# Alibaba-Gemini-Lab/Gemini-SEAL

Measured on AMD Instinct MI355X. Metric: ciphertext multiply+relinearize/s (BFV N=2^15, 8 primes, bit-exact PARITY mode), higher is better.
Workload: dtype u64

## Files before the change

### gemini-seal_amd/csrc/api.cpp

```cpp
#include "../../include/sealhip.h"

#include <algorithm>
#include <cmath>
#include <cstdio>
#include <cstdlib>
#include <functional>
#include <vector>
#include <cstring>
#include <new>

#include "blake2xb.hpp"
#include "engine.hpp"
#include "evalmod_plan.hpp"
#include "homdft_plan.hpp"
#include "poly_plan.hpp"

using namespace sealhip;

namespace sealhip
{
    void wire_set_parms_id(Engine &e, int k, const std::uint64_t *id);
    void wire_peek(const void *bytes, std::size_t len, sealhip_ciphertext_info *info);
    void wire_load(Engine &e, const void *bytes, std::size_t len, sealhip_ciphertext_info *info, u64 *dst,
                   std::size_t capacity_words);
// ... 623 lines not shown
                          first ? "" : ", ", kv.first.c_str(), kv.second.launches, kv.second.ms, kv.second.units);
            out += buf;
            first = false;
        }
        out += "}";
        if (out.size() + 1 > capacity)
            throw std::invalid_argument("capacity too small");
        std::memcpy(json, out.c_str(), out.size() + 1);
    });
}

long sealhip_debug_ntt_table(sealhip_context *ctx, uint32_t prime_index, uint32_t kind, uint64_t *out_host,
                             size_t capacity)
{
    REQUIRE_PTR(ctx);
    REQUIRE_PTR(out_host);
    return guarded([&] {
        Engine &e = *ctx->engine;
        if (static_cast<int>(prime_index) >= e.n_primes() || kind > 3)
            throw std::invalid_argument("table index out of range");
        if (capacity < e.n)
            throw std::invalid_argument("capacity too small");
        const HostNttTables &tb = e.tables[prime_index];
        if (tb.fwd.empty())
            throw std::invalid_argument("this prime has no NTT tables");
        const std::vector<u64> v = tb.reference_table(static_cast<int>(kind));
        std::memcpy(out_host, v.data(), v.size() * sizeof(u64));
    });
}

long sealhip_debug_rns_constants(sealhip_context *ctx, uint32_t k, uint32_t which, uint64_t *out_host,
                                 size_t capacity, size_t *written)
{
    REQUIRE_PTR(ctx);
    REQUIRE_PTR(out_host);
    REQUIRE_PTR(written);
    return guarded([&] {
        Engine &e = *ctx->engine;
        check_level(e, k);
        const HostRnsTool &r = *e.level_host(static_cast<int>(k)).host_rns;
        std::vector<u64> v;
        switch (which)
        {
        case 0: v = r.Bsk; break;
        case 1: v = r.inv_prod_q_mod_Bsk; break;
        case 2: v = r.prod_q_mod_Bsk; break;
        case 3: v = r.inv_m_tilde_mod_Bsk; break;
        case 4: v = r.prod_B_mod_q; break;
        case 5: v = r.inv_q_last_mod_q; break;
        case 6: v = { r.inv_prod_q_mod_m_tilde, r.inv_prod_B_mod_m_sk, r.m_sk, r.gamma }; break;
        case 7: v = r.q_to_Bsk.matrix; break;
        case 8: v = r.B_to_q.matrix; break;
        case 9: v = r.q_to_Bsk.inv_punct; break;
        case 10: v = r.B_to_q.inv_punct; break;
        case 11: v = r.q_to_m_tilde.matrix; break;
        case 12: v = r.B_to_m_sk.matrix; break;
        default: throw std::invalid_argument("unknown constant selector");
        }
        if (capacity < v.size())
            throw std::invalid_argument("capacity too small");
        std::memcpy(out_host, v.data(), v.size() * sizeof(u64));
        *written = v.size();
    });
}

long sealhip_debug_bfv_multiply_plan(sealhip_context *ctx, uint32_t k, uint32_t size_a, uint32_t size_b, int32_t square,
                                     int32_t *out)
{
    REQUIRE_PTR(ctx);
    REQUIRE_PTR(out);
    return guarded([&] {
        Engine &e = *ctx->engine;
        check_level(e, k);
        if (size_a < 2 || size_b < 2 || size_a + size_b - 1 > 16)
            throw std::invalid_argument("encrypted1 or encrypted2 is not valid for encryption parameters");
        const BfvMulPlan p = plan_bfv_multiply(e, static_cast<int>(k), static_cast<int>(size_a), static_cast<int>(size_b),
                                               square != 0);
        const int32_t v[13] = { p.k, p.B, p.nB, p.square, p.redc_small, p.gather, p.defer, p.fused_tensor, p.tensor_apx,
                                p.lift_top, p.lift_kernel, p.floor_kernel, p.deferred_top };
        std::memcpy(out, v, sizeof v);
    });
}

long sealhip_debug_behz_dot_split(sealhip_context *ctx, uint32_t k, int32_t *out)
{
    REQUIRE_PTR(ctx);
    REQUIRE_PTR(out);
    return guarded([&] {
        Engine &e = *ctx->engine;
        check_level(e, k);
        if (e.scheme != 1)
            throw std::invalid_argument("BFV contexts only");
        if (e.device >= 0)
        {
            *out = e.level(static_cast<int>(k)).h_rns.dot_split;
            return;
        }
        const HostRnsTool &r = *e.level_host(static_cast<int>(k)).host_rns;
        const u64 max_q = *std::max_element(r.q.begin(), r.q.end()), max_b = *std::max_element(r.Bsk.begin(), r.Bsk.end());
        *out = bounds::behz_select_split(static_cast<int>(k), max_q, max_b);
    });
}

long sealhip_ntt_negacyclic_harvey_lazy(sealhip_context *ctx, uint64_t *data, size_t count, uint32_t k, uint32_t base)
{
    REQUIRE_PTR(ctx);
    REQUIRE_PTR(data);
    return guarded([&] { ntt_entry(ctx, data, count, k, base, false, 0); });
}
long sealhip_ntt_negacyclic_harvey(sealhip_context *ctx, uint64_t *data, size_t count, uint32_t k, uint32_t base)
{
    REQUIRE_PTR(ctx);
    REQUIRE_PTR(data);
    return guarded([&] { ntt_entry(ctx, data, count, k, base, false, kNttCanonical); });
}
long sealhip_inverse_ntt_negacyclic_harvey_lazy(sealhip_context *ctx, uint64_t *data, size_t count, uint32_t k,
                                                uint32_t base)
{
    REQUIRE_PTR(ctx);
    REQUIRE_PTR(data);
    return guarded([&] { ntt_entry(ctx, data, count, k, base, true, 0); });
}
long sealhip_inverse_ntt_negacyclic_harvey(sealhip_context *ctx, uint64_t *data, size_t count, uint32_t k,
                                           uint32_t base)
{
    REQUIRE_PTR(ctx);
    REQUIRE_PTR(data);
    return guarded([&] { ntt_entry(ctx, data, count, k, base, true, kNttCanonical); });
}

long sealhip_dyadic_product_coeffmod(sealhip_context *ctx, const uint64_t *a, const uint64_t *b, size_t count,
                                     uint32_t k, uint32_t base, uint64_t *result)
{
    REQUIRE_PTR(ctx);
    REQUIRE_PTR(a);
    REQUIRE_PTR(b);
    REQUIRE_PTR(result);
    return guarded([&] { poly_entry(ctx, PolyOp::Dyadic, a, b, 0, result, count, k, base); });
}
long sealhip_multiply_poly_scalar_coeffmod(sealhip_context *ctx, const uint64_t *a, size_t count, uint32_t k,
                                           uint32_t base, uint64_t scalar, uint64_t *result)
{
    REQUIRE_PTR(ctx);
    REQUIRE_PTR(a);
    REQUIRE_PTR(result);
    return guarded([&] { poly_entry(ctx, PolyOp::Scalar, a, a, scalar, result, count, k, base); });
}
long sealhip_add_poly_coeffmod(sealhip_context *ctx, const uint64_t *a, const uint64_t *b, size_t count, uint32_t k,
                               uint32_t base, uint64_t *result)
{
    REQUIRE_PTR(ctx);
    REQUIRE_PTR(a);
    REQUIRE_PTR(b);
    REQUIRE_PTR(result);
    return guarded([&] { poly_entry(ctx, PolyOp::Add, a, b, 0, result, count, k, base); });
}
long sealhip_sub_poly_coeffmod(sealhip_context *ctx, const uint64_t *a, const uint64_t *b, size_t count, uint32_t k,
                               uint32_t base, uint64_t *result)
{
    REQUIRE_PTR(ctx);
    REQUIRE_PTR(a);
    REQUIRE_PTR(b);
    REQUIRE_PTR(result);
    return guarded([&] { poly_entry(ctx, PolyOp::Sub, a, b, 0, result, count, k, base); });
}
long sealhip_negate_poly_coeffmod(sealhip_context *ctx, const uint64_t *a, size_t count, uint32_t k, uint32_t base,
// ... 3225 lines not shown
```

### gemini-seal_amd/csrc/engine.hpp

```cpp
#pragma once

#include <hip/hip_runtime.h>

#include <cstddef>
#include <array>
#include <atomic>
#include <cstdint>
#include <functional>
#include <map>
#include <memory>
#include <mutex>
#include <stdexcept>
#include <string>
#include <cstdlib>
#include <vector>

#include "devmath.hpp"
#include "ntt_bounds.hpp"
#include "ntt_select.hpp"
#include "hostmath.hpp"
#include "pool_scratch.hpp"
#include "held_workspace.hpp"
struct sealhip_kswitch_key;

// ... 280 lines not shown
        int n_primes() const
        {
            return static_cast<int>(tables.size());
        }
        LevelTools &level(int k);
        LevelTools &level_host(int k);
        LevelTools &level_rescale(int k);
        const std::uint32_t *galois_table(std::uint32_t elt);
        void ws_reset() const
        {
            Lane &l = lane();
            l.ws_used = l.ws_floor;
        }
        u64 *ws_alloc(std::size_t words) const;
        void ws_reserve(std::size_t bytes) const;
        RowMap map_for(int k, unsigned base);
        int rows_for(int k, unsigned base);
    };

    struct HipError : std::runtime_error
    {
        hipError_t code;
        HipError(hipError_t c, const char *what) : std::runtime_error(what), code(c)
        {}
    };
#define SEALHIP_CHECK(expr)                                                                          \
    do                                                                                               \
    {                                                                                                \
        hipError_t _e = (expr);                                                                      \
        if (_e != hipSuccess)                                                                        \
            throw ::sealhip::HipError(_e, (std::string(#expr) + ": " + hipGetErrorString(_e)).c_str()); \
    } while (0)
    inline void check(hipError_t err, const char *what)
    {
        if (err != hipSuccess)
            throw HipError(err, (std::string(what) + ": " + hipGetErrorString(err)).c_str());
    }

    inline std::size_t pad256(std::size_t words)
    {
        return (words * sizeof(u64) + 255) & ~static_cast<std::size_t>(255);
    }
    struct Carver
    {
        char *base;
        std::size_t at = 0;
        u64 *take(std::size_t words)
        {
            u64 *p = reinterpret_cast<u64 *>(base + at);
            at += pad256(words);
            return p;
        }
    };

    constexpr int kThreads = 256;
    inline unsigned grid_for(std::size_t work_items, std::size_t max_blocks = 256u * 16u)
    {
        const std::size_t blocks = (work_items + kThreads - 1) / kThreads;
        return static_cast<unsigned>(blocks < max_blocks ? (blocks ? blocks : 1) : max_blocks);
    }

    struct ProfScope
    {
        const Engine &e;
        ProfScope(const Engine &eng, const char *tag, double units) : e(eng)
        {
            if (e.lane().prof_on)
                e.prof_begin(tag, units);
        }
        ~ProfScope()
        {
            if (e.lane().prof_on)
                e.prof_end();
        }
    };

    hipError_t ntt_init_kernels();
    hipError_t ntt_butterfly_rate(const Engine &e, int kind, int prime_id, double *butterflies_per_s);
    hipError_t launch_ntt(const Engine &e, u64 *data, std::size_t nrows, const RowMap &map, bool inverse, int flags);
    bool ntt_can_gather(const Engine &e);
    bool ntt_strict_top_done_ok(const Engine &e, const RowMap &map);
    hipError_t launch_ntt_gather(const Engine &e, u64 *data, std::size_t nrows, const RowMap &map, const NttSource &src,
                                 int flags);

    enum class PolyOp
    {
        Dyadic,
        Add,
        Sub,
        Negate,
        Scalar,
        Mod63
    };
    hipError_t launch_poly_op(const Engine &e, PolyOp op, const u64 *a, const u64 *b, u64 scalar, u64 *r,
                              std::size_t nrows, const RowMap &map);
    hipError_t launch_tensor_product(const Engine &e, const u64 *a, int sa, std::size_t a_stride, const u64 *b, int sb,
                                     std::size_t b_stride, u64 *out, std::size_t out_stride, std::size_t count,
                                     const RowMap &map, bool square = false);
    hipError_t launch_fill_rows(const Engine &e, u64 *dst, const u64 *row_values, int rows, std::size_t count);
    constexpr int kDotGroup = bounds::kDotGroupTerms;
    struct DotTerms
    {
        const u64 *a[kDotGroup];
        const u64 *b[kDotGroup];
        int n;
    };
    hipError_t launch_tensor_dot(const Engine &e, const DotTerms &terms, std::size_t a_stride, std::size_t b_stride, u64 *out01,
                                 std::size_t out01_stride, u64 *out2, std::size_t out2_stride, std::size_t count,
                                 const RowMap &map, bool reduce_on_load, bool add_partial);
    constexpr int kLinGroup = bounds::kLinGroupTerms, kLinTile = bounds::kLinTileSums;
    struct LinTerms
    {
        const u64 *x[kLinGroup];
        int n;
    };
    hipError_t launch_lincomb(const Engine &e, const LinTerms &terms, int size, std::size_t x_stride, const u64 *w,
                              std::size_t w_sum_stride, const u64 *constant, int const_mode, u64 *out, std::size_t out_sum_stride,
                              int n_sums, std::size_t count, const RowMap &map, bool add_partial, std::size_t flag_sum_stride);
    constexpr int kLinLevelsTile = bounds::kLinLevelsTileSums;
    struct LinLevelTerms
    {
        const u64 *x[kLinGroup];
        unsigned char rows[kLinGroup];
        unsigned char size[kLinGroup];
        int n;
    };
    hipError_t launch_lincomb_levels(const Engine &e, const LinLevelTerms &terms, int size, std::size_t out_stride, const u64 *w,
                                     std::size_t w_sum_stride, const u64 *constant, int const_mode, u64 *out,
                                     std::size_t out_sum_stride, int n_sums, std::size_t count, const RowMap &map,
                                     bool add_partial, std::size_t flag_sum_stride);
    hipError_t launch_poly_tables(const Engine &e, int k, const u64 *coeffs, std::size_t n_coeffs, std::size_t ms, u64 *w,
                                  u64 *constant);
    constexpr int kPutWords = 256;
    hipError_t launch_put_words(const Engine &e, u64 *dst, const u64 *words, std::size_t n);
    hipError_t launch_copy_rows(const Engine &e, const u64 *src, std::size_t src_poly_stride, u64 *dst,
                                std::size_t dst_poly_stride, std::size_t npolys, int rows);

    hipError_t launch_fastbconv_m_tilde(const Engine &e, const RnsDev *d, const RnsDev &h, const u64 *in,
                                        std::size_t in_stride, u64 *out, std::size_t out_stride, std::size_t count);
    hipError_t launch_sm_mrq(const Engine &e, const RnsDev *d, const RnsDev &h, const u64 *in, std::size_t in_stride,
                             u64 *out, std::size_t out_stride, std::size_t count);
    constexpr int kBehzGeneric = 32;
    constexpr int kBehzStepwise = 64;
    struct BfvMulPlan
    {
        int k, B, nB;
        bool square;
        bool redc_small;
        bool gather;
        bool defer;
        bool fused_tensor;
        bool tensor_apx;
        bool lift_top;
        int lift_kernel;
        int floor_kernel;
        int deferred_top;
    };
    BfvMulPlan plan_bfv_multiply(Engine &e, int k, int sa, int sb, bool square);

    bool bfv_lift_can_apply_top(const Engine &e, int k, bool redc_small);
    hipError_t launch_bfv_lift(const Engine &e, const RnsDev *d, const RnsDev &h, const u64 *in, std::size_t in_stride,
                               u64 *out, std::size_t out_stride, std::size_t count, const BfvMulPlan &plan);
    hipError_t launch_fast_floor(const Engine &e, const RnsDev *d, const RnsDev &h, const u64 *in,
                                 std::size_t in_stride, u64 *out, std::size_t out_stride, std::size_t count,
                                 int mul_t);
    hipError_t launch_fastbconv_sk(const Engine &e, const RnsDev *d, const RnsDev &h, const u64 *in,
                                   std::size_t in_stride, u64 *out, std::size_t out_stride, std::size_t count);
    hipError_t launch_bfv_floor_sk(const Engine &e, const RnsDev *d, const RnsDev &h, const u64 *in,
                                   std::size_t in_stride, u64 *out, std::size_t out_stride, std::size_t count,
                                   const BfvMulPlan &plan);
    bool ntt_can_defer_top(const Engine &e, int k);
    bool ntt_can_fuse_moddown(const Engine &e, int k, u64 p_special);
    hipError_t launch_intt_from(const Engine &e, u64 *data, const u64 *src, std::size_t src_poly_stride, std::size_t nrows,
                                const RowMap &map, int flags);
    hipError_t launch_intt_tensor(const Engine &e, u64 *data, const u64 *x, std::size_t item_stride, std::size_t poly_stride,
                                  int kb, std::size_t nrows, const RowMap &map, int flags, bool square = false);
    hipError_t launch_divround_bfv(const Engine &e, const RnsDev *d, const RnsDev &h, const u64 *in,
                                   std::size_t in_stride, u64 *out, std::size_t out_stride, std::size_t count,
                                   int out_rows);
    hipError_t launch_rescale_pre(const Engine &e, const RnsDev *d, const RnsDev &h, u64 *last,
                                  std::size_t last_stride, u64 *temp, std::size_t temp_stride, std::size_t count);
    hipError_t launch_rescale_post(const Engine &e, const RnsDev *d, const RnsDev &h, const u64 *in,
                                   std::size_t in_stride, const u64 *temp, std::size_t temp_stride, u64 *out,
                                   std::size_t out_stride, std::size_t count);

    enum class CtLinearOp
    {
        Add,
        Sub,
        Negate,
        MulPlain
    };
    hipError_t launch_ct_linear(const Engine &e, CtLinearOp op, const u64 *a, int sa, const u64 *b, int sb,
                                std::size_t b_item_stride, u64 *out, std::size_t count, const RowMap &map);
    hipError_t launch_nonzero_words(const Engine &e, const u64 *data, std::size_t item_stride, std::size_t words,
                                    std::size_t count, unsigned *flags);
    hipError_t launch_nonzero_tail(const Engine &e, const u64 *ct, std::size_t item_words, std::size_t skip_words,
                                   std::size_t count, unsigned *flags);
    struct SinkScope
    {
        Engine &e;
        Lane &l;
        bool on;
        size_t count;
        bool cleared = false;
        SinkScope(Engine &eng, size_t n) : e(eng), l(eng.lane()), on(l.tsink != nullptr), count(n)
        {
            if (on && count > l.tsink_cap)
                throw std::invalid_argument("the transparency sink is smaller than this batch");
        }
        void clear()
        {
            if (on && !cleared && count)
                SEALHIP_CHECK(hipMemsetAsync(l.tsink, 0, count * sizeof(unsigned), l.stream));
            cleared = true;
            l.tsink_base = 0;
        }
        void begin()
        {
            clear();
            if (on)
                l.tsink_cur = l.tsink;
        }
        void arm()
        {
            begin();
        }
        void read_pass(const u64 *result, uint32_t size, size_t poly_words, size_t n)
        {
            clear();
            if (on && size >= 2 && n)
                check(launch_nonzero_tail(e, result, poly_words * size, poly_words, n, l.tsink), "transparency");
        }
        ~SinkScope()
        {
            l.tsink_cur = l.tsink_arm = nullptr;
            l.tsink_base = 0;
        }
    };
    hipError_t launch_out_of_range(const Engine &e, const u64 *ct, std::size_t item_words, std::size_t count,
                                   const RowMap &map, unsigned *flags);
    hipError_t launch_plain_lift(const Engine &e, const u64 *plain, std::size_t plain_stride, u64 *out, std::size_t nplains,
                                 const RowMap &map, u64 t);
    hipError_t launch_plain_lift_centered(const Engine &e, const u64 *plain, std::size_t coeff_count, std::size_t plain_stride,
                                          u64 *out, std::size_t nplains, const RowMap &map, u64 t);
    hipError_t launch_galois(const Engine &e, const u64 *in, u64 *out, std::size_t nrows, const RowMap &map,
                             std::uint32_t elt, const std::uint32_t *table );

    hipError_t launch_ks_modup(const Engine &e, const KsDev *d, const KsDev &h, const u64 *coeff,
                               std::size_t coeff_stride, u64 *ext, std::size_t ext_stride,
                               std::size_t ext_digit_stride, std::size_t count, int only_digit);
    hipError_t launch_ks_mac(const Engine &e, const KsDev *d, const KsDev &h, const u64 *target,
                             std::size_t target_stride, const u64 *ext, std::size_t ext_stride,
                             std::size_t ext_digit_stride, const u64 *key, u64 *prod, std::size_t prod_stride,
                             std::size_t count, int j0 = 0, int j1 = -1);
    hipError_t launch_ks_moddown_pre(const Engine &e, const KsDev *d, const KsDev &h, const u64 *prod,
                                     std::size_t prod_stride, u64 *temp, std::size_t temp_stride, std::size_t npolys);
    hipError_t launch_ks_moddown_bfv(const Engine &e, const KsDev *d, const KsDev &h, const u64 *prod,
                                     std::size_t prod_stride, u64 *ct, std::size_t ct_item_stride, std::size_t npolys,
                                     bool top_deferred, const u64 *c0_src = nullptr, std::size_t c0_stride = 0);
    hipError_t launch_ks_moddown_post(const Engine &e, const KsDev *d, const KsDev &h, u64 *prod,
                                      std::size_t prod_stride, const u64 *temp, std::size_t temp_stride, u64 *ct,
                                      std::size_t ct_item_stride, std::size_t npolys, int add_into_ct,
                                      const u64 *c0_src = nullptr, std::size_t c0_stride = 0);
    hipError_t launch_ks_rescale_fold(const Engine &e, const KsRescaleDev *d, const KsRescaleDev &h, const u64 *base,
                                      std::size_t base_stride, u64 *acc, std::size_t acc_stride, std::size_t npolys);
    hipError_t launch_ks_moddown_rescale_pre(const Engine &e, const KsRescaleDev *d, const KsRescaleDev &h, const u64 *acc,
                                             std::size_t acc_stride, u64 *temp, std::size_t npolys);
    hipError_t launch_ks_moddown_rescale_post(const Engine &e, const KsRescaleDev *d, const KsRescaleDev &h, const u64 *base,
                                              std::size_t base_stride, const u64 *acc, std::size_t acc_stride, const u64 *temp,
                                              u64 *out, std::size_t npolys);

    constexpr int kHoistMaxElts = 16;
    struct HoistElts
    {
        int n;
        std::uint32_t elt[kHoistMaxElts];
        const std::uint32_t *table[kHoistMaxElts];
        const u64 *key[kHoistMaxElts];
    };
    hipError_t launch_hoist_mac(const Engine &e, const KsDev *d, const KsDev &h, const u64 *target,
                                std::size_t target_stride, const u64 *ext, std::size_t ext_stride,
                                std::size_t ext_digit_stride, const HoistElts &elts, u64 *prod, std::size_t prod_stride,
                                std::size_t count);
    hipError_t launch_hoist_galois_c0(const Engine &e, const u64 *ct, std::size_t ct_stride, u64 *out, std::size_t count,
                                      const RowMap &map_q, const HoistElts &elts, bool ntt_form);
    struct HoistDotElts
    {
        int n;
        const std::uint32_t *table[kHoistMaxElts];
        const u64 *key[kHoistMaxElts];
        const u64 *w[kHoistMaxElts];
    };
    hipError_t launch_hoist_dot_mac(const Engine &e, const KsDev *d, const KsDev &h, const u64 *target,
                                    std::size_t target_stride, const u64 *ext, std::size_t ext_stride,
                                    std::size_t ext_digit_stride, const HoistDotElts &elts, std::size_t w_sum_stride, u64 *acc,
                                    std::size_t acc_stride, std::size_t count, std::size_t n_sums, bool add);
    hipError_t launch_hoist_dot_base(const Engine &e, const u64 *cn, const HoistDotElts &elts, std::size_t w_sum_stride,
                                     u64 *out, std::size_t out_sum_stride, int k, std::size_t count, std::size_t n_sums,
                                     bool add);

    struct HoistGiantElts
    {
        int n;
        const std::uint32_t *table[kHoistMaxElts];
        const u64 *key[kHoistMaxElts];
        const u64 *inb[kHoistMaxElts];
        const u64 *ext[kHoistMaxElts];
        const u64 *accj[kHoistMaxElts];
    };
    hipError_t launch_hoist_giant_mac(const Engine &e, const KsDev *d, const KsDev &h, const HoistGiantElts &elts,
                                      std::size_t inb_stride, std::size_t ext_stride, std::size_t ext_digit_stride,
                                      std::size_t accj_stride, u64 *acc, std::size_t acc_stride, std::size_t count, bool add);
    struct HoistGiantBases
    {
        int n;
        const std::uint32_t *table[kHoistMaxElts];
        const u64 *base[kHoistMaxElts];
    };
    hipError_t launch_hoist_giant_base(const Engine &e, const HoistGiantBases &elts, u64 *out, int k, std::size_t count,
                                       bool add);

    struct HostBatchIO
    {
        struct In
        {
            const u64 *const *ptrs;
            std::size_t words;
        };
        struct Out
        {
            u64 *const *ptrs;
            std::size_t words;
        };
        std::vector<In> in;
        std::vector<Out> out;
        std::size_t tmp_words = 0;
    };
// ... 276 lines not shown
```

### gemini-seal_amd/csrc/keyswitch.hip

```cpp
#include <cstdlib>
#include "engine.hpp"

namespace sealhip
{
    namespace
    {
        __device__ __forceinline__ const u64 *modup_block(const KsDev *d, int j)
        {
            const int rows = d->k + d->nsp;
            return d->modup + static_cast<std::size_t>(j) * (2 * d->nsp + rows * d->nsp);
        }

        __global__ __launch_bounds__(kThreads) void ks_modup_kernel(const KsDev *__restrict__ d,
                                                                    const PrimeDev *__restrict__ primes,
                                                                    const u64 *__restrict__ coeff,
                                                                    std::size_t coeff_stride, u64 *__restrict__ ext,
                                                                    std::size_t ext_stride,
                                                                    std::size_t ext_digit_stride, std::size_t count,
                                                                    int logn, int only_digit)
        {
            const std::size_t i = blockIdx.x * static_cast<std::size_t>(blockDim.x) + threadIdx.x;
            const std::size_t item = i >> logn;
            if (item >= count)
                return;
// ... 85 lines not shown
            const int my_digit = r < k ? r / nsp : -1;
            const u64 *pext = ext + item * ext_stride + static_cast<std::size_t>(r) * N + c;
            const u64 *pkey = key + static_cast<std::size_t>(rns_idx) * N + c;
            const std::size_t key_comp = static_cast<std::size_t>(n_total) * N;
            u64 lo0 = 0, hi0 = 0, lo1 = 0, hi1 = 0;
            for (int j = j0; j < j1; j++)
            {
                const u64 x = j == my_digit ? target[item * target_stride + static_cast<std::size_t>(r) * N + c]
                                            : pext[static_cast<std::size_t>(j) * ext_digit_stride];
                const u64 k0 = pkey[(2 * static_cast<std::size_t>(j)) * key_comp];
                const u64 k1 = pkey[(2 * static_cast<std::size_t>(j) + 1) * key_comp];
                mac128(lo0, hi0, x, k0);
                mac128(lo1, hi1, x, k1);
            }
            const PrimeDev &P = primes[rns_idx];
            u64 *pp = prod + item * prod_stride + static_cast<std::size_t>(r) * N + c;
            pp[0] = barrett_reduce_128(lo0, hi0, P.p, P.cr0, P.cr1);
            pp[static_cast<std::size_t>(rows) * N] = barrett_reduce_128(lo1, hi1, P.p, P.cr0, P.cr1);
        }

        template <int ND>
        __global__ __launch_bounds__(kThreads) void ks_mac_items_kernel(const KsDev *__restrict__ d,
                                                                        const PrimeDev *__restrict__ primes,
                                                                        const u64 *__restrict__ target,
                                                                        std::size_t target_stride,
                                                                        const u64 *__restrict__ ext,
                                                                        std::size_t ext_stride,
                                                                        std::size_t ext_digit_stride,
                                                                        const u64 *__restrict__ key,
                                                                        u64 *__restrict__ prod, std::size_t prod_stride,
                                                                        std::size_t count, int logn, std::size_t group)
        {
            const std::size_t N = static_cast<std::size_t>(1) << logn;
            const int k = d->k, nsp = d->nsp, rows = k + nsp, n_total = d->n_total;
            const std::size_t i = blockIdx.x * static_cast<std::size_t>(blockDim.x) + threadIdx.x;
            const std::size_t c = i & (N - 1);
            const std::size_t rr = i >> logn;
            const int r = static_cast<int>(rr % rows);
            const std::size_t item0 = (rr / rows) * group;
            if (item0 >= count)
                return;
            const std::size_t item1 = item0 + group < count ? item0 + group : count;
            const int rns_idx = d->row_prime[r];
            const int my_digit = r < k ? r / nsp : -1;
            const std::size_t row_off = static_cast<std::size_t>(r) * N + c;
            const u64 *pkey = key + static_cast<std::size_t>(rns_idx) * N + c;
            const std::size_t key_comp = static_cast<std::size_t>(n_total) * N;
            u64 k0[ND], k1[ND], x[ND], xn[ND];
#pragma unroll
            for (int j = 0; j < ND; j++)
            {
                k0[j] = pkey[(2 * static_cast<std::size_t>(j)) * key_comp];
                k1[j] = pkey[(2 * static_cast<std::size_t>(j) + 1) * key_comp];
            }
            auto load_x = [&](u64(&dst)[ND], std::size_t item) {
#pragma unroll
                for (int j = 0; j < ND; j++)
                    dst[j] = j == my_digit ? target[item * target_stride + row_off]
                                           : ext[item * ext_stride + static_cast<std::size_t>(j) * ext_digit_stride + row_off];
            };
            load_x(x, item0);
            const PrimeDev &P = primes[rns_idx];
            const u64 p = P.p, cr0 = P.cr0, cr1 = P.cr1;
            for (std::size_t item = item0; item < item1; item++)
            {
                if (item + 1 < item1)
                    load_x(xn, item + 1);
                u64 lo0 = 0, hi0 = 0, lo1 = 0, hi1 = 0;
#pragma unroll
                for (int j = 0; j < ND; j++)
                {
                    mac128(lo0, hi0, x[j], k0[j]);
                    mac128(lo1, hi1, x[j], k1[j]);
                }
                u64 *pp = prod + item * prod_stride + row_off;
                store_stream(pp, barrett_reduce_128(lo0, hi0, p, cr0, cr1));
                store_stream(pp + static_cast<std::size_t>(rows) * N, barrett_reduce_128(lo1, hi1, p, cr0, cr1));
#pragma unroll
                for (int j = 0; j < ND; j++)
                    x[j] = xn[j];
            }
        }

        __global__ __launch_bounds__(kThreads) void ks_moddown_pre_kernel(const KsDev *__restrict__ d,
                                                                          const PrimeDev *__restrict__ primes,
                                                                          const u64 *__restrict__ prod,
                                                                          std::size_t prod_stride,
                                                                          u64 *__restrict__ temp,
                                                                          std::size_t temp_stride, std::size_t npolys,
                                                                          int logn)
        {
            const std::size_t i = blockIdx.x * static_cast<std::size_t>(blockDim.x) + threadIdx.x;
            const std::size_t poly = i >> logn;
            if (poly >= npolys)
                return;
            const std::size_t N = static_cast<std::size_t>(1) << logn;
            const std::size_t c = i & (N - 1);
            const int k = d->k, nsp = d->nsp;
            const u64 *sp = prod + poly * prod_stride + static_cast<std::size_t>(k) * N + c;
            u64 *pt = temp + poly * temp_stride + c;
            if (nsp == 1)
            {
                const PrimeDev &S = primes[d->row_prime[k]];
                const u64 v = neg_mod(barrett_reduce_63(sp[0], S.p, S.cr1), S.p);
                for (int q = 0; q < k; q++)
                {
                    const PrimeDev &Q = primes[d->row_prime[q]];
                    pt[q * N] = barrett_reduce_63(v, Q.p, Q.cr1);
                }
                return;
            }
            for (int q = 0; q < k; q++)
            {
                const PrimeDev &Q = primes[d->row_prime[q]];
                u64 lo = 0, hi = 0;
                for (int j = 0; j < nsp; j++)
                {
                    const u64 pj = primes[d->row_prime[k + j]].p;
                    const u64 y = mulmod_shoup(sp[j * N], d->inv_hat[j], d->inv_hat_shoup[j], pj);
                    mac128(lo, hi, y, d->neg_hat[q * nsp + j]);
                }
                pt[q * N] = barrett_reduce_128(lo, hi, Q.p, Q.cr0, Q.cr1);
            }
        }

        __global__ __launch_bounds__(kThreads) void ks_moddown_post_kernel(const KsDev *__restrict__ d,
                                                                           const PrimeDev *__restrict__ primes,
                                                                           u64 *__restrict__ prod,
                                                                           std::size_t prod_stride,
                                                                           const u64 *__restrict__ temp,
                                                                           std::size_t temp_stride,
                                                                           u64 *__restrict__ ct,
                                                                           std::size_t ct_item_stride,
                                                                           std::size_t npolys, int logn,
                                                                           int add_into_ct, const u64 *__restrict__ c0_src,
                                                                           std::size_t c0_stride, unsigned *__restrict__ tflags)
        {
            const std::size_t N = static_cast<std::size_t>(1) << logn;
            const int k = d->k;
            const std::size_t i = blockIdx.x * static_cast<std::size_t>(blockDim.x) + threadIdx.x;
            const std::size_t c = i & (N - 1);
            const std::size_t rr = i >> logn;
            const int q = static_cast<int>(rr % k);
            const std::size_t poly = rr / k;
            if (poly >= npolys)
                return;
            const PrimeDev &Q = primes[d->row_prime[q]];
            u64 *pp = prod + poly * prod_stride + static_cast<std::size_t>(q) * N + c;
            const u64 v = mulmod_shoup(*pp + temp[poly * temp_stride + static_cast<std::size_t>(q) * N + c], d->invP[q],
                                       d->invP_shoup[q], Q.p);
            if (add_into_ct)
            {
                u64 *pc = ct + (poly >> 1) * ct_item_stride + ((poly & 1) * static_cast<std::size_t>(k) + q) * N + c;
                u64 w;
                if (!c0_src)
                    w = add_mod(v, *pc, Q.p);
                else
                    w = (poly & 1) ? v : add_mod(v, c0_src[(poly >> 1) * c0_stride + static_cast<std::size_t>(q) * N + c], Q.p);
                *pc = w;
                if (poly & 1)
                    note_nonzero(tflags, poly >> 1, w);
            }
            else
                *pp = v;
        }

// ... 144 lines not shown
                u64 z[ND1];
#pragma unroll
                for (int a = 0; a < ND1; a++)
                    z[a] = rescale_z(d, primes, a, dp[a * N], slo, shi);
                const u64 v = shi;
                for (int r = 0; r < k - 1; r++)
                {
                    const PrimeDev &Q = primes[r];
                    const u64 *hat = d->hat + static_cast<std::size_t>(r) * ND1;
                    u64 lo = d->neg_half[r], hi = 0;
#pragma unroll
                    for (int a = 0; a < ND1; a++)
                        mac128(lo, hi, z[a], hat[a]);
                    mac128(lo, hi, v, d->neg_D[r]);
                    pt[r * N] = barrett_reduce_128(lo, hi, Q.p, Q.cr0, Q.cr1);
                }
            }
            else
            {
                for (int a = 0; a < nd1; a++)
                    rescale_z(d, primes, a, dp[a * N], slo, shi);
                const u64 v = shi;
                for (int r = 0; r < k - 1; r++)
                {
                    const PrimeDev &Q = primes[r];
                    const u64 *hat = d->hat + static_cast<std::size_t>(r) * nd1;
                    u64 lo = d->neg_half[r], hi = 0, s0 = 0, s1 = 0;
                    for (int a = 0; a < nd1; a++)
                        mac128(lo, hi, rescale_z(d, primes, a, dp[a * N], s0, s1), hat[a]);
                    mac128(lo, hi, v, d->neg_D[r]);
                    pt[r * N] = barrett_reduce_128(lo, hi, Q.p, Q.cr0, Q.cr1);
                }
            }
        }

        __global__ __launch_bounds__(kThreads) void ks_moddown_rescale_post_kernel(const KsRescaleDev *__restrict__ d,
                                                                                   const PrimeDev *__restrict__ primes,
                                                                                   const u64 *__restrict__ base,
                                                                                   std::size_t base_stride,
                                                                                   const u64 *__restrict__ acc,
                                                                                   std::size_t acc_stride,
                                                                                   const u64 *__restrict__ temp, u64 *__restrict__ out,
                                                                                   std::size_t npolys, int logn,
                                                                                   unsigned *__restrict__ tflags)
        {
            const std::size_t N = static_cast<std::size_t>(1) << logn;
            const int k = d->k, kk = k - 1;
            const std::size_t i = blockIdx.x * static_cast<std::size_t>(blockDim.x) + threadIdx.x;
            const std::size_t c = i & (N - 1);
            const std::size_t rr = i >> logn;
            const int r = static_cast<int>(rr % kk);
            const std::size_t poly = rr / kk;
            if (poly >= npolys)
                return;
            const PrimeDev &Q = primes[r];
            const std::size_t row = static_cast<std::size_t>(r) * N + c;
            const u64 b = base[(poly >> 1) * base_stride + (poly & 1) * static_cast<std::size_t>(k) * N + row];
            const u64 s = mul_add_mod(b, d->P_mod_q[r], acc[poly * acc_stride + row], Q.p, Q.cr0, Q.cr1);
            const std::size_t o = poly * static_cast<std::size_t>(kk) * N + row;
            const u64 w = mulmod_shoup(sub_mod(s, temp[o], Q.p), d->invD[r], d->invD_shoup[r], Q.p);
            store_stream(out + o, w);
            if (poly & 1)
                note_nonzero(tflags, poly >> 1, w);
        }

        inline unsigned blocks_for(std::size_t lanes)
        {
            return static_cast<unsigned>((lanes + kThreads - 1) / kThreads);
        }
    }

    hipError_t launch_ks_modup(const Engine &e, const KsDev *d, const KsDev &, const u64 *coeff,
                               std::size_t coeff_stride, u64 *ext, std::size_t ext_stride,
                               std::size_t ext_digit_stride, std::size_t count, int only_digit)
    {
        if (!count)
            return hipSuccess;
        ProfScope prof(e, "ks_modup", 0);
        ks_modup_kernel<<<blocks_for(count << e.logn), kThreads, 0, e.lane().stream>>>(
            d, e.d_primes, coeff, coeff_stride, ext, ext_stride, ext_digit_stride, count, e.logn, only_digit);
        return hipGetLastError();
    }

    hipError_t launch_ks_mac(const Engine &e, const KsDev *d, const KsDev &h, const u64 *target,
                             std::size_t target_stride, const u64 *ext, std::size_t ext_stride,
                             std::size_t ext_digit_stride, const u64 *key, u64 *prod, std::size_t prod_stride,
                             std::size_t count, int j0, int j1)
    {
        if (!count)
            return hipSuccess;
        if (j1 < 0)
            j1 = h.nd;
        if (j0 < 0 || j0 > j1 || j1 > h.nd)
            return hipErrorInvalidValue;
        const bool all_digits = j0 == 0 && j1 == h.nd;
        const u64 *tg = target;
        const std::size_t lanes = (count * static_cast<std::size_t>(h.k + h.nsp)) << e.logn;
        ProfScope prof(e, "ks_mac", 0);
        const std::size_t key_bytes = (2ull * h.nd * (h.k + h.nsp)) << (e.logn + 3);
        const std::size_t cap = key_bytes > (std::size_t(48) << 20) ? 64 : 16;
        std::size_t mac_group = 8;
        for (std::size_t g = cap; g > 8; g >>= 1)
            if ((((count + g - 1) / g * static_cast<std::size_t>(h.k + h.nsp)) << e.logn) / kThreads >= 4096)
            {
                mac_group = g;
                break;
            }
        const std::size_t groups = (count + mac_group - 1) / mac_group;
        const std::size_t glanes = (groups * static_cast<std::size_t>(h.k + h.nsp)) << e.logn;
#define SEALHIP_KS_MAC(ND)                                                                                          \
    case ND:                                                                                                        \
        ks_mac_items_kernel<ND><<<blocks_for(glanes), kThreads, 0, e.lane().stream>>>(                                     \
            d, e.d_primes, tg, target_stride, ext, ext_stride, ext_digit_stride, key, prod, prod_stride, count,    \
            e.logn, mac_group);                                                                                     \
        break;
        switch (count >= 16 && all_digits ? h.nd : 0)
        {
            SEALHIP_KS_MAC(1)
            SEALHIP_KS_MAC(2)
            SEALHIP_KS_MAC(3)
            SEALHIP_KS_MAC(4)
            SEALHIP_KS_MAC(5)
            SEALHIP_KS_MAC(6)
            SEALHIP_KS_MAC(7)
            SEALHIP_KS_MAC(8)
            SEALHIP_KS_MAC(9)
            SEALHIP_KS_MAC(10)
            SEALHIP_KS_MAC(11)
            SEALHIP_KS_MAC(12)
            SEALHIP_KS_MAC(13)
            SEALHIP_KS_MAC(14)
            SEALHIP_KS_MAC(15)
            SEALHIP_KS_MAC(16)
        default:
            ks_mac_kernel<<<blocks_for(lanes), kThreads, 0, e.lane().stream>>>(d, e.d_primes, tg, target_stride, ext, ext_stride,
                                                                        ext_digit_stride, key, prod, prod_stride, count,
                                                                        e.logn, j0, j1);
        }
#undef SEALHIP_KS_MAC
        return hipGetLastError();
    }

    hipError_t launch_ks_moddown_pre(const Engine &e, const KsDev *d, const KsDev &, const u64 *prod,
                                     std::size_t prod_stride, u64 *temp, std::size_t temp_stride, std::size_t npolys)
    {
        if (!npolys)
            return hipSuccess;
        ProfScope prof(e, "ks_moddown_pre", 0);
        ks_moddown_pre_kernel<<<blocks_for(npolys << e.logn), kThreads, 0, e.lane().stream>>>(
            d, e.d_primes, prod, prod_stride, temp, temp_stride, npolys, e.logn);
        return hipGetLastError();
    }

    hipError_t launch_ks_moddown_bfv(const Engine &e, const KsDev *d, const KsDev &h, const u64 *prod,
                                     std::size_t prod_stride, u64 *ct, std::size_t ct_item_stride, std::size_t npolys,
                                     bool top_deferred, const u64 *c0_src, std::size_t c0_stride)
    {
        if (!npolys)
            return hipSuccess;
        const std::size_t lanes = npolys << (e.logn - 1);
        ProfScope prof(e, "ks_moddown_bfv", 0);
#define SEALHIP_MODDOWN_BFV(DEFER_, ONE_)                                                                            \
    ks_moddown_bfv_kernel<DEFER_, ONE_><<<blocks_for(lanes), kThreads, 0, e.lane().stream>>>(                              \
        d, e.d_primes, prod, prod_stride, ct, ct_item_stride, npolys, e.logn, c0_src, c0_stride, e.lane().tsink_arm)
        if (top_deferred && h.nsp == 1)
            SEALHIP_MODDOWN_BFV(true, true);
        else if (top_deferred)
            SEALHIP_MODDOWN_BFV(true, false);
        else if (h.nsp == 1)
            SEALHIP_MODDOWN_BFV(false, true);
        else
            SEALHIP_MODDOWN_BFV(false, false);
#undef SEALHIP_MODDOWN_BFV
        return hipGetLastError();
    }

    hipError_t launch_ks_moddown_post(const Engine &e, const KsDev *d, const KsDev &h, u64 *prod,
                                      std::size_t prod_stride, const u64 *temp, std::size_t temp_stride, u64 *ct,
                                      std::size_t ct_item_stride, std::size_t npolys, int add_into_ct, const u64 *c0_src,
                                      std::size_t c0_stride)
    {
        if (!npolys)
            return hipSuccess;
        const std::size_t lanes = (npolys * static_cast<std::size_t>(h.k)) << e.logn;
        ProfScope prof(e, "ks_moddown_post", 0);
        ks_moddown_post_kernel<<<blocks_for(lanes), kThreads, 0, e.lane().stream>>>(
            d, e.d_primes, prod, prod_stride, temp, temp_stride, ct, ct_item_stride, npolys, e.logn, add_into_ct, c0_src, c0_stride,
            add_into_ct ? e.lane().tsink_arm : nullptr);
        return hipGetLastError();
    }

    hipError_t launch_ks_rescale_fold(const Engine &e, const KsRescaleDev *d, const KsRescaleDev &, const u64 *base,
// ... 51 lines not shown
```

### gemini-seal_amd/csrc/ntt.hip

```cpp
#include <cstdlib>
#include <stdexcept>

#include "ntt_half.hpp"

namespace sealhip
{
    namespace
    {
        constexpr int kTileBitsMax = 13;

        __device__ __forceinline__ int pad_index(int l)
        {
            return l + (l >> 4);
        }

        template <int DIR>
        __global__ __launch_bounds__(512, 4) void ntt_pass_kernel(u64 *__restrict__ data,
                                                               const PrimeDev *__restrict__ primes, RowMap map,
                                                               NttPass ps)
        {
            extern __shared__ u64 lds[];
            const int tid = threadIdx.x;
            const int nthreads = blockDim.x;
            const int t = ps.t, c = ps.c, b_lo = ps.b_lo, logn = ps.logn;
// ... 421 lines not shown
                               reinterpret_cast<const void *>(&butterfly_rate_kernel<4>), reinterpret_cast<const void *>(&butterfly_rate_kernel<5>) };
        if ((err = hipFuncSetAttribute(fns[kind], hipFuncAttributeMaxDynamicSharedMemorySize, static_cast<int>(lds))) != hipSuccess)
        {
            (void)hipEventDestroy(a);
            (void)hipEventDestroy(b);
            (void)hipFree(sink);
            return err;
        }
        const auto launch = [&](int n) {
            switch (kind)
            {
            case 0: butterfly_rate_kernel<0><<<blocks, 512, lds, st>>>(sink, P, n); break;
            case 1: butterfly_rate_kernel<1><<<blocks, 512, lds, st>>>(sink, P, n); break;
            case 2: butterfly_rate_kernel<2><<<blocks, 512, lds, st>>>(sink, P, n); break;
            case 3: butterfly_rate_kernel<3><<<blocks, 512, lds, st>>>(sink, P, n); break;
            case 4: butterfly_rate_kernel<4><<<blocks, 512, lds, st>>>(sink, P, n); break;
            default: butterfly_rate_kernel<5><<<blocks, 512, lds, st>>>(sink, P, n); break;
            }
        };
        launch(iters / 8);
        (void)hipEventRecord(a, st);
        launch(iters);
        launch(iters);
        (void)hipEventRecord(b, st);
        err = hipStreamSynchronize(st);
        float ms = 0;
        if (err == hipSuccess)
            err = hipEventElapsedTime(&ms, a, b);
        (void)hipEventDestroy(a);
        (void)hipEventDestroy(b);
        (void)hipFree(sink);
        if (err != hipSuccess)
            return err;
        *butterflies_per_s = 2.0 * blocks * 512.0 * iters * 32.0 / (ms / 1e3);
        return hipGetLastError();
    }

    hipError_t ntt_init_kernels()
    {
        const int max_lds = ((1 << kTileBitsMax) + (1 << (kTileBitsMax - 4))) * 8;
        hipError_t err = hipFuncSetAttribute(reinterpret_cast<const void *>(&ntt_pass_kernel<0>),
                                             hipFuncAttributeMaxDynamicSharedMemorySize, max_lds);
        if (err != hipSuccess)
            return err;
        err = hipFuncSetAttribute(reinterpret_cast<const void *>(&ntt_pass_kernel<1>),
                                  hipFuncAttributeMaxDynamicSharedMemorySize, max_lds);
        if (err == hipSuccess)
            err = ntt_fwd_half_init();
        if (err == hipSuccess)
            err = ntt_inv_half_init();
        return err;
    }

    bool ntt_can_defer_top(const Engine &e, int k)
    {
        return e.use_half_kernel && e.logn >= 14 && e.logn <= 16 && k <= 32;
    }

    bool ntt_can_fuse_moddown(const Engine &e, int k, u64 p_special)
    {
        if (!fp64_enabled() || !ntt_can_gather(e) || e.logn < 15 || p_special >= kFpPrimeBound)
            return false;
        for (int r = 0; r < k; r++)
            if (e.key_moduli[r] >= kFpPrimeBound)
                return false;
        return true;
    }

    bool ntt_strict_top_done_ok(const Engine &e, const RowMap &map)
    {
        if (!e.use_half_kernel || e.logn < 14 || e.logn > 16 || exact_fwd())
            return false;
        for (int r = 0; r < map.rows; r++)
            if (map.prime[r] != kSkipRow && !bounds::fwd_dense_admits(e.tables[map.prime[r]].p, e.logn))
                return false;
        return true;
    }

    bool ntt_can_gather(const Engine &e)
    {
        return e.use_half_kernel && e.logn >= 14 && e.logn <= 16;
    }

    hipError_t launch_ntt_gather(const Engine &e, u64 *data, size_t nrows, const RowMap &map, const NttSource &src,
                                 int flags)
    {
        if (!ntt_can_gather(e))
            return hipErrorInvalidValue;
        if (e.mode_strict)
            flags |= kNttStrict;
        if (nrows == 0)
            return hipSuccess;
        return ntt_fwd_half(e, data, nrows, map, flags, src);
    }

    hipError_t launch_intt_from(const Engine &e, u64 *data, const u64 *src, std::size_t src_poly_stride, size_t nrows,
                                const RowMap &map, int flags)
    {
        if (!(e.use_half_kernel && e.logn >= 14 && e.logn <= 16))
            return hipErrorInvalidValue;
        if (nrows == 0)
            return hipSuccess;
        return ntt_inv_half(e, data, nrows, map, flags, src, src_poly_stride);
    }

    hipError_t launch_intt_tensor(const Engine &e, u64 *data, const u64 *x, std::size_t item_stride, std::size_t poly_stride,
                                  int kb, size_t nrows, const RowMap &map, int flags, bool square)
    {
        if (!(e.use_half_kernel && e.logn >= 14 && e.logn <= 16) || map.rows != 3 * kb)
            return hipErrorInvalidValue;
        if (nrows == 0)
            return hipSuccess;
        return ntt_inv_tensor(e, data, nrows, map, flags, x, item_stride, poly_stride, kb, square);
    }

    hipError_t launch_ntt(const Engine &e, u64 *data, size_t nrows, const RowMap &map, bool inverse, int flags)
    {
        if (nrows == 0)
            return hipSuccess;
        if (e.mode_strict)
            flags |= kNttStrict;
        if (e.use_half_kernel && e.logn >= 14 && e.logn <= 16)
            return inverse ? ntt_inv_half(e, data, nrows, map, flags) : ntt_fwd_half(e, data, nrows, map, flags, NttSource{});
        if (e.logn > kTileBitsMax)
            return hipErrorInvalidValue;
        const NttPlan plan = plan_ntt(e.logn, inverse, flags);
        return inverse ? launch_dir<1>(e, data, nrows, map, plan) : launch_dir<0>(e, data, nrows, map, plan);
    }
}
```

### gemini-seal_amd/csrc/ntt_bounds.hpp

```cpp
#pragma once
#include <cstdint>

namespace sealhip
{
    namespace bounds
    {
        using u64 = unsigned long long;
        using u128 = unsigned __int128;

        constexpr int kMinHalfLogn = 14, kMaxHalfLogn = 16;
        constexpr int kMaxPrimeBits = 61;
        constexpr u128 kWord = static_cast<u128>(1) << 64;
        constexpr long double kFpLimit = 9007199254740992.0L;

        constexpr u64 max_prime_of_bits(int bits)
        {
            return (bits >= 64 ? ~u64(0) : (u64(1) << bits) - 1);
        }
        constexpr u64 max_ntt_prime_of_bits(int bits, int logn)
        {
            return bits > logn + 1 ? (u64(1) << bits) - (u64(1) << (logn + 1)) + 1 : 0;
        }

        constexpr int kInvLazyProductMult = 4;
// ... 61 lines not shown
                          inv_lazy_prime_bits(16, 1) == 60,
                      "dense lazy inverse: primes below 2^60 in every shape");
        static_assert(inv_lazy_max_shift(16, 1) == 3, "dense lazy inverse: values entering a layer are below 8p");

        constexpr int kFwdApxLevel = 2;
        static_assert(kFwdApxLevel == 1 || kFwdApxLevel == 2, "approximate-quotient form");
        constexpr int quotient_shortfall(int level)
        {
            return level == 0 ? 1 : (level == 1 ? 2 : 3);
        }
        constexpr int kFwdApxGrowth = quotient_shortfall(kFwdApxLevel) + 1;
        constexpr u128 fwd_int_peak(int logn, u64 p, int in_mult, bool apx, bool skip_last_barrett)
        {
            const u128 g = static_cast<u128>(apx ? kFwdApxGrowth : 2) * p;
            u128 bound = static_cast<u128>(in_mult) * p, peak = bound;
            for (int l = 0; l < logn; l++)
            {
                u128 u = bound;
                if (l == logn - 1 && !skip_last_barrett)
                    u = static_cast<u128>(2) * p;
                const u128 out = u + g;
                peak = out > peak ? out : peak;
                bound = out;
            }
            return peak;
        }
        constexpr int fwd_lazy_prime_bits(int logn)
        {
            int bits = 0;
            for (int b = 1; b <= kMaxPrimeBits; b++)
                if (fwd_int_peak(logn, max_prime_of_bits(b), 2, true, true) < kWord)
                    bits = b;
            return bits;
        }
        static_assert(kFwdApxLevel != 1 || (fwd_lazy_prime_bits(14) == 58 && fwd_lazy_prime_bits(16) == 58),
                      "level 1: kNttAnyRep / kNttApprox / unreduced mod-up: primes below 2^58 (50p at log n = 16)");
        static_assert(kFwdApxLevel != 2 || (fwd_lazy_prime_bits(14) == 58 && fwd_lazy_prime_bits(15) == 58 && fwd_lazy_prime_bits(16) == 57),
                      "level 2: 58p / 62p below 2^64 for primes below 2^58 at log n = 14 / 15; 66p at log n = 16: below 2^57");
        constexpr bool fwd_lazy_admits(u64 p, int logn)
        {
            return logn >= kMinHalfLogn && logn <= kMaxHalfLogn && p <= max_prime_of_bits(fwd_lazy_prime_bits(logn));
        }
        constexpr int kCanonInMult = 4;
        constexpr int fwd_canon_output_mult(int logn)
        {
            return kCanonInMult + kFwdApxGrowth * logn;
        }
        constexpr bool fwd_canon_admits(u64 p, int logn)
        {
            return logn >= kMinHalfLogn && logn <= kMaxHalfLogn && fwd_lazy_admits(p, logn) &&
                   fwd_int_peak(logn, p, kCanonInMult, true, true) < kWord;
        }
        constexpr int fwd_apx_output_mult(int logn, bool anyrep)
        {
            return anyrep ? 2 + kFwdApxGrowth * logn : 2 + kFwdApxGrowth;
        }

        constexpr int kFwdDenseInMult = 4;
        constexpr bool fwd_dense_reduce_before_round(int r)
        {
            return r == 2 || r == 3;
        }
        constexpr int fwd_dense_peak_mult(int logn)
        {
            int b = kFwdDenseInMult + 2, peak = b;
            for (int r = 1; r <= 4; r++)
            {
                if (fwd_dense_reduce_before_round(r))
                    b = 2;
                const int layers = r <= 3 ? 4 : logn - 13;
                for (int l = 0; l < layers; l++)
                    b += 2;
                peak = b > peak ? b : peak;
            }
            return peak;
        }
        constexpr bool fwd_dense_admits(u64 p, int logn)
        {
            return logn >= kMinHalfLogn && logn <= kMaxHalfLogn && p < (u64(1) << 60) &&
                   small_quot_admits(p, fwd_dense_peak_mult(logn)) && static_cast<u128>(fwd_dense_peak_mult(logn)) * p <= kWord;
        }
        static_assert(fwd_dense_peak_mult(14) == 14 && fwd_dense_peak_mult(15) == 14 && fwd_dense_peak_mult(16) == 16,
                      "dense forward schedule: 14p after round 1, at most 16p after the final round at N = 2^16");

        constexpr bool tensor_redc_ok(u64 p, int operand_mult, int np)
        {
            const u128 ob = static_cast<u128>(operand_mult) * p;
            if (ob > (static_cast<u128>(1) << 61) || np > 2)
                return false;
            return (ob - 1) * (ob - 1) * np <= static_cast<u128>(p) * kWord;
        }
        constexpr int tensor_prime_bits(int operand_mult)
        {
            int bits = 0;
            for (int b = 1; b <= kMaxPrimeBits; b++)
                if (tensor_redc_ok(max_prime_of_bits(b), operand_mult, 2))
                    bits = b;
            return bits;
        }
        constexpr int kTensorPrimeBits4p = tensor_prime_bits(4);
        constexpr int kTensorPrimeBits2p = tensor_prime_bits(2);
        static_assert(kTensorPrimeBits4p == 59, "fused tensor product on [0, 4p) operands: ciphertext primes below 2^59");
        static_assert(kTensorPrimeBits2p == 60, "... on [0, 2p) operands (kNttReduceOut rows): the 60-bit Bsk primes");
        constexpr bool tensor_admits_4p(u64 p)
        {
            return p <= max_prime_of_bits(kTensorPrimeBits4p);
        }
        constexpr bool tensor_admits_2p(u64 p)
        {
            return p <= max_prime_of_bits(kTensorPrimeBits2p);
        }
        constexpr int kTensorPrimeBitsApx = tensor_prime_bits(fwd_apx_output_mult(kMaxHalfLogn, false));
        static_assert(kTensorPrimeBitsApx == (kFwdApxLevel == 2 ? 57 : 58), "fused tensor product on approximate-quotient rows");
        constexpr bool tensor_admits_apx(u64 p)
        {
            return p <= max_prime_of_bits(kTensorPrimeBitsApx);
        }

        constexpr long double kFpSlack = 1.0L + 0x1p-40L;
        constexpr long double fp_mul_bound(long double y, long double p)
        {
            return 0.5L * p + 3.0L * 0x1p-53L * y * p * kFpSlack;
        }
        constexpr long double fp_reduce_bound(long double x, long double p)
        {
            return 0.5L * p + x * 0x1p-51L + 1.0L;
        }
        constexpr bool fp_fwd_reduce_before_layer(int i)
        {
            return i == 5 || i == 10;
        }
        constexpr long double fp_fwd_peak(int logn, long double p, long double in_bound)
        {
            long double b = in_bound, peak = in_bound;
            b = b + fp_mul_bound(b, p);
            peak = b > peak ? b : peak;
            b = fp_reduce_bound(b, p);
            for (int i = 0; i < logn - 1; i++)
            {
                if (fp_fwd_reduce_before_layer(i))
                    b = fp_reduce_bound(b, p);
                b = b + fp_mul_bound(b, p);
                peak = b > peak ? b : peak;
            }
            return peak;
        }
        constexpr bool fp_inv_reduce_after_layer(int T, int l)
        {
            return l % 4 == 1 && l != T - 1;
        }
        constexpr long double fp_inv_peak(int T, long double p)
        {
            long double b = 2.0L * p, peak = b;
            for (int l = 0; l < T; l++)
            {
                const long double s = 2.0L * b;
                peak = s > peak ? s : peak;
                const long double r = fp_mul_bound(s, p);
                b = s > r ? s : r;
                if (fp_inv_reduce_after_layer(T, l))
                    b = fp_reduce_bound(b, p);
            }
            return peak;
        }
        constexpr int fp_prime_bits()
        {
// ... 268 lines not shown
```

### gemini-seal_amd/csrc/ntt_fwd.hip

```cpp
#include <cstring>
#include <utility>

#include "ntt_half.hpp"

namespace sealhip
{
    namespace
    {
        template <int STRICT>
        constexpr int kApx = STRICT == kSchedApprox ? bounds::kFwdApxLevel : 0;
        constexpr int kFinalZeroPairs = 2;
        template <int T, int STRICT>
        constexpr int kFinalApx = (kApx<STRICT> == 2 && (T - 12) == 2) ? 1 : kApx<STRICT>;
        template <int STRICT>
        __device__ __forceinline__ u64 fwd_addend(u64 two_p, u64 neg_p)
        {
            if constexpr (STRICT != kSchedApprox)
                return two_p;
            u64 a = two_p << 1;
            asm("" : "+s"(a));
            return a;
        }


// ... 462 lines not shown
                        };
                        top(lo[i].x, hi[i].x);
                        top(lo[i].y, hi[i].y);
                    }
                }
                if constexpr (REDUCE == kTreatNegSpecial)
                {
#pragma unroll
                    for (int i = 0; i < kLoadBatch; i++)
                    {
                        const auto red = [&](u64 v) {
                            if constexpr (STRICT == kSchedFp64)
                            {
                                const double P = fp_of(aux_p), r = fp_canonical(fp_from_u64(v), P, fp_of(aux_cr1));
                                return fp_bits(r != 0.0 ? P - r : 0.0);
                            }
                            const u64 r = barrett_reduce_63(v, aux_p, aux_cr1);
                            return r ? aux_p - r : 0;
                        };
                        lo[i].x = red(lo[i].x);
                        lo[i].y = red(lo[i].y);
                        hi[i].x = red(hi[i].x);
                        hi[i].y = red(hi[i].y);
                    }
                }
                if constexpr (REDUCE == kTreatBarrett || REDUCE == kTreatCondSub)
                {
                    const u64 p = STRICT == kSchedFp64 ? static_cast<u64>(fp_of(two_p)) : 0 - neg_p;
                    const auto red = [&](u64 v) {
                        if constexpr (REDUCE == kTreatCondSub)
                            return v >= p ? v - p : v;
                        else
                            return barrett_reduce_63(v, p, cr1);
                    };
#pragma unroll
                    for (int i = 0; i < kLoadBatch; i++)
                    {
                        lo[i].x = red(lo[i].x);
                        lo[i].y = red(lo[i].y);
                        hi[i].x = red(hi[i].x);
                        hi[i].y = red(hi[i].y);
                    }
                }
#pragma unroll
                for (int i = 0; i < kLoadBatch; i += 2)
                {
                    const int s = (batch * kLoadBatch + i) * 2;
                    u64 u[4] = {lo[i].x, lo[i].y, lo[i + 1].x, lo[i + 1].y};
                    u64 y[4] = {hi[i].x, hi[i].y, hi[i + 1].x, hi[i + 1].y};
                    if constexpr (STRICT == kSchedFp64)
                    {
#pragma unroll
                        for (int j = 0; j < 4; j++)
                        {
                            if constexpr (REDUCE != kTreatNegSpecial && REDUCE != kTreatNegSpecialTop && REDUCE != kTreatModDownStore)
                            {
                                u[j] = fp_bits(fp_from_u64(u[j]));
                                y[j] = fp_bits(fp_from_u64(y[j]));
                            }
                            fp_butterfly_fwd(u[j], y[j], W1.x, fp_of(two_p), fp_of(neg_p));
                            x[s + j] = HALF ? y[j] : u[j];
                        }
                        continue;
                    }
                    const u64 w[4] = {W1.x, W1.x, W1.x, W1.x}, ws[4] = {W1.y, W1.y, W1.y, W1.y};
                    if (STRICT == kSchedHarvey)
                    {
#pragma unroll
                        for (int j = 0; j < 4; j++)
                            u[j] = u[j] >= two_p ? u[j] - two_p : u[j];
                    }
                    if constexpr (kApx<STRICT> == 2)
                        butterflies_fwd_apx2<true, 4>(u, y, w, ws, neg_p, fwd_addend<STRICT>(two_p, neg_p), zp.z);
                    else
                        butterflies_fwd_hs<true, 4, kApx<STRICT>>(u, y, w, ws, neg_p, fwd_addend<STRICT>(two_p, neg_p));
#pragma unroll
                    for (int j = 0; j < 4; j++)
                        x[s + j] = HALF ? y[j] : u[j];
                }
                __builtin_amdgcn_sched_barrier(0);
            }
        }

        template <int T>
        __device__ __forceinline__ void h_store_rows(const u64 (&x)[32], u64 *__restrict__ halfp, int tid)
        {
            const int jb = Arr<T, 1>::tid_index(tid);
#pragma unroll
            for (int s = 0; s < 32; s += 2)
                store_nt(halfp + jb + Arr<T, 1>::slot_index(s), x[s], x[s + 1]);
        }

        template <int T>
        __device__ __forceinline__ void h_store_moddown(const u64 (&x)[32], int tid, const u64 *__restrict__ prod_half,
                                                        u64 *__restrict__ ct_half, const u64 *__restrict__ c0_half, bool add_ct,
                                                        u64 inv_p, u64 inv_p_shoup, u64 p, unsigned *__restrict__ tflag)
        {
            const int jb = Arr<T, 1>::tid_index(tid);
            u64 nz = 0;
#pragma unroll
            for (int b = 0; b < 32; b += 8)
            {
                ulonglong2 pr[4], cc[4];
#pragma unroll
                for (int i = 0; i < 4; i++)
                {
                    const int off = jb + Arr<T, 1>::slot_index(b + 2 * i);
                    pr[i] = *reinterpret_cast<const ulonglong2 *>(prod_half + off);
                    if (c0_half)
                        cc[i] = *reinterpret_cast<const ulonglong2 *>(c0_half + off);
                    else if (add_ct)
                        cc[i] = *reinterpret_cast<const ulonglong2 *>(ct_half + off);
                }
#pragma unroll
                for (int i = 0; i < 4; i++)
                {
                    const int off = jb + Arr<T, 1>::slot_index(b + 2 * i);
                    u64 v0 = mulmod_shoup(pr[i].x + x[b + 2 * i], inv_p, inv_p_shoup, p);
                    u64 v1 = mulmod_shoup(pr[i].y + x[b + 2 * i + 1], inv_p, inv_p_shoup, p);
                    if (c0_half || add_ct)
                    {
                        v0 = add_mod(v0, cc[i].x, p);
                        v1 = add_mod(v1, cc[i].y, p);
                    }
                    store_nt(ct_half + off, v0, v1);
                    nz |= v0 | v1;
                }
            }
            note_nonzero(tflag, 0, nz);
        }

        template <int LOGN, int STRICT, int REDUCE>
        __global__ __launch_bounds__(1 << (LOGN - 6), 4) void ntt_fwd_half_kernel(
            u64 *__restrict__ data, const PrimeDev *__restrict__ primes, RowMap map, std::size_t nrows, int flags,
            unsigned *__restrict__ tickets, unsigned *__restrict__ timeout_flag, unsigned spin_limit, NttSource src,
            std::size_t chunk, LiveSlots live)
        {
            constexpr int T = LOGN - 1;
            constexpr int N = 1 << LOGN;
            extern __shared__ u64 lds[];
            const int wave_base = __builtin_amdgcn_readfirstlane(static_cast<int>(threadIdx.x) & ~63);
            int half, position;
            std::size_t poly;
            if (!half_block_map(blockIdx.x, nrows / map.rows, live.n, chunk, poly, position, half,
                                (flags & kNttPolyMajor) ? ((flags >> 16) & 0xFF) : 0))
                return;
            const std::size_t row = poly * map.rows + live.slot[position];
            const unsigned short pid = map.prime[row % map.rows];
            const PrimeDev P = primes[pid];
            constexpr bool FP = STRICT == kSchedFp64;
            const u64 p = P.p, two_p = FP ? fp_bits(P.p_d) : P.two_p, rdp = P.rdp;
            const u64 *tw = FP ? reinterpret_cast<const u64 *>(P.fwd_d) : P.fwd;
            u64 *rowp = data + (row << LOGN);
            u64 x[32];

            const u64 neg_p = FP ? fp_bits(P.pinv_d) : 0 - p;
            const u64 *srcp = rowp;
            if (src.base[0])
            {
                const unsigned short code = src.code[row % map.rows];
                if (code != kSkipRow)
                {
                    const int b = code >> 15;
                    srcp = src.base[b] + (row / map.rows) * src.poly_stride[b] +
                           (static_cast<std::size_t>(code & 0x3FFF) << LOGN);
                }
            }
            if constexpr (REDUCE == kTreatReduceOutTopDone)
            {
                const int jb1 = Arr<T, 1>::tid_index(fresh_tid(wave_base));
#pragma unroll
                for (int s = 0; s < 32; s += 2)
                {
                    const ulonglong2 v = *reinterpret_cast<const ulonglong2 *>(rowp + (half << T) + jb1 + Arr<T, 1>::slot_index(s));
                    x[s] = v.x;
                    x[s + 1] = v.y;
                }
            }
            else if (half)
                h_load_top<T, STRICT, 1, REDUCE>(x, srcp, tw, fresh_tid(wave_base), two_p, neg_p, P.cr1, src.aux_p, src.aux_cr1, src.aux_top);
            else
                h_load_top<T, STRICT, 0, REDUCE>(x, srcp, tw, fresh_tid(wave_base), two_p, neg_p, P.cr1, src.aux_p, src.aux_cr1, src.aux_top);
            const int gbase = half << T;
            u64 w0[kIL], ws0[kIL];
            RoundStage<T, 1, STRICT, true, 0>::load(w0, ws0, tw, gbase, N);
            if constexpr (FP)
                fp_reduce_all(x, two_p, neg_p);
            ZeroPairs zp;
            if constexpr (kApx<STRICT> == 2)
                zp.init();
            RoundPipe<T, 1, STRICT, true>::run(x, w0, ws0, tw, gbase, N, two_p, neg_p, zp);
            const int jb2 = gbase + Arr<T, 2>::tid_index(fresh_tid(wave_base));
            RoundStage<T, 2, STRICT, false, 0>::load(w0, ws0, tw, jb2, N);
            __builtin_amdgcn_sched_barrier(0);
            h_exchange<T, 1, 2>(x, lds, fresh_tid(wave_base));
            if (fresh_tid(wave_base) == 0 && tickets && !(flags & kNttDebugNoSignal))
                __hip_atomic_fetch_add(&tickets[row], 1u, __ATOMIC_RELAXED, __HIP_MEMORY_SCOPE_AGENT);
            if constexpr (kApx<STRICT> == 2)
                zp.init();
            RoundPipe<T, 2, STRICT, false>::run(x, w0, ws0, tw, jb2, N, two_p, neg_p, zp);
            const int jb3 = gbase + Arr<T, 3>::tid_index(fresh_tid(wave_base));
            RoundStage<T, 3, STRICT, false, 0>::load(w0, ws0, tw, jb3, N);
            __builtin_amdgcn_sched_barrier(0);
            h_exchange<T, 2, 3>(x, lds, fresh_tid(wave_base));
            if constexpr (kApx<STRICT> == 2)
                zp.init();
            RoundPipe<T, 3, STRICT, false>::run(x, w0, ws0, tw, jb3, N, two_p, neg_p, zp);
            const int jb4 = gbase + Arr<T, 4>::tid_index(fresh_tid(wave_base));
            u64x2 tg0[FinalStage<T>::SG * FinalStage<T>::NTW];
            if constexpr (FinalStage<T>::PIPE)
            {
                StageTw<T, 0, 0, STRICT == kSchedFp64>::load(tg0, tw, jb4, N);
                __builtin_amdgcn_sched_barrier(0);
            }
            h_exchange<T, 3, 4>(x, lds, fresh_tid(wave_base));
            static_assert(!bounds::fp_fwd_reduce_before_layer(12) && !bounds::fp_fwd_reduce_before_layer(13) &&
                              !bounds::fp_fwd_reduce_before_layer(14),
                          "the final round runs without a reduction (the schedule reduces inside rounds 2 and 3)");
            const auto wait_for_sibling = [&] {
                if ((fresh_tid(wave_base) & 63) == 0 && tickets)
                {
                    unsigned spins = 0;
                    while (__hip_atomic_load(&tickets[row], __ATOMIC_RELAXED, __HIP_MEMORY_SCOPE_AGENT) < 2u)
                    {
                        __builtin_amdgcn_s_sleep(8);
                        if (++spins > spin_limit)
                        {
                            __hip_atomic_store(timeout_flag, 1u, __ATOMIC_RELAXED, __HIP_MEMORY_SCOPE_SYSTEM);
                            break;
                        }
                    }
                }
            };
            constexpr bool XCH = kStoreExchange<T, REDUCE>;
            constexpr int SX = XCH ? 1 : (kStoreSwap<T, REDUCE> ? 2 : 0);
            if constexpr (!XCH)
                wait_for_sibling();
            const int fin = ((flags & kNttCanonical) ? 1 : 0) | (((flags & kNttAnyRep) || STRICT == kSchedDense) ? 2 : 0) | ((flags & kNttSmallQuot) ? 4 : 0);
            const u64 rdp_fin =
                ((STRICT == kSchedApprox && (flags & kNttSmallQuot)) || STRICT == kSchedDense) ? static_cast<u64>(__float_as_uint(small_quot_const(p))) : rdp;
            constexpr bool ROUT = REDUCE == kTreatReduceOut || REDUCE == kTreatReduceOutTopDone;
            if constexpr (kFinalApx<T, STRICT> == 2)
                zp.init();
            if constexpr (FinalStage<T>::PIPE)
                FinalPipe<T, STRICT, ROUT, SX, 0>::run(x, tg0, tw, rowp, jb4, N, p, two_p, neg_p, rdp_fin, fin, zp);
            else
                FinalGroups<T, STRICT, 0, 1 << (5 - (T - 12)), ROUT, SX>::run(x, tw, rowp, jb4, N, p, two_p, neg_p, rdp_fin, fin, zp);
            if constexpr (XCH)
            {
                h_exchange<T, 4, 1>(x, lds, fresh_tid(wave_base));
                wait_for_sibling();
                if constexpr (REDUCE == kTreatModDownStore)
                {
                    const std::size_t pl = row / map.rows, q = row % map.rows;
                    typedef const __attribute__((address_space(4))) u64 *kc_t;
                    const u64 ip = ((kc_t)src.md.inv_p)[q], ips = ((kc_t)src.md.inv_p_shoup)[q];
                    const u64 *prod_half = src.md.prod + pl * src.md.prod_stride + (q << LOGN) + gbase;
                    u64 *ct_half = src.md.ct + (pl >> 1) * src.md.ct_stride + (((pl & 1) * map.rows + q) << LOGN) + gbase;
                    const u64 *c0_half =
                        (src.md.c0_src && !(pl & 1)) ? src.md.c0_src + (pl >> 1) * src.md.c0_stride + (q << LOGN) + gbase : nullptr;
                    h_store_moddown<T>(x, fresh_tid(wave_base), prod_half, ct_half, c0_half, src.md.c0_src == nullptr, ip, ips, P.p,
                                       (src.md.tflags && (pl & 1)) ? src.md.tflags + (pl >> 1) : nullptr);
                }
                else
                    h_store_rows<T>(x, rowp + gbase, fresh_tid(wave_base));
            }
        }

        using FwdKernel = void (*)(u64 *, const PrimeDev *, RowMap, std::size_t, int, unsigned *, unsigned *, unsigned, NttSource,
                                   std::size_t, LiveSlots);
        template <int LOGN, int I>
        FwdKernel fwd_kernel()
        {
            if constexpr (fwd_instance_at(LOGN, kFwdInstances[I]))
                return &ntt_fwd_half_kernel<LOGN, kFwdInstances[I].sched, kFwdInstances[I].treatment>;
            else
                return nullptr;
        }
        template <int LOGN, int... I>
        const FwdKernel *fwd_kernels(std::integer_sequence<int, I...>)
        {
            static const FwdKernel table[] = { fwd_kernel<LOGN, I>()... };
            return table;
        }
        template <int LOGN>
        const FwdKernel *fwd_kernels()
        {
            return fwd_kernels<LOGN>(std::make_integer_sequence<int, kFwdInstanceCount>{});
        }

        template <int LOGN>
        hipError_t launch_half(const Engine &e, u64 *data, std::size_t nrows, const RowMap &map, int flags,
                               const NttSource &src)
        {
            constexpr int T = LOGN - 1;
            const std::size_t lds_bytes = static_cast<std::size_t>(hpad(1 << (T - 1))) * 8;
            if (nrows % map.rows != 0)
                return hipErrorInvalidValue;
            if (fp64_enabled() && (flags & (kNttAnyRep | kNttCanonical)) != 0 && (flags & kNttReduceOut) == 0 && !src.base[0])
            {
                RowMap a, b;
                if (split_by_fp(e, map, a, b))
                {
                    const hipError_t err = launch_half<LOGN>(e, data, nrows, a, flags, src);
                    return err != hipSuccess ? err : launch_half<LOGN>(e, data, nrows, b, flags, src);
                }
            }
            const LiveSlots live = live_slots(map);
            if (live.n == 0)
                return hipSuccess;
            const std::size_t chunk = ((nrows / map.rows) * live.n + 7) / 8;
            const std::size_t blocks = chunk * 16;
            if (blocks > 0x7fffffffull)
                return hipErrorInvalidValue;
            u64 live_p[kMaxRows];
            FwdFacts f{};
            f.logn = LOGN;
            f.flags = flags;
            f.live = live_p;
            f.live_n = live.n;
            f.gathers = src.base[0] != nullptr;
            f.all_gathered = f.same_source = f.key_moduli_fp = true;
            for (int i = 0; i < live.n; i++)
            {
                live_p[i] = e.tables[map.prime[live.slot[i]]].p;
                if (f.gathers)
                {
                    f.all_gathered = f.all_gathered && src.code[live.slot[i]] != kSkipRow;
                    f.same_source = f.same_source && ((src.code[live.slot[i]] ^ src.code[live.slot[0]]) & ~kSrcReduce) == 0;
                }
            }
            for (std::size_t i = 0; f.gathers && f.key_moduli_fp && i < e.key_moduli.size(); i++)
                f.key_moduli_fp = e.key_moduli[i] < bounds::kFpInputBound;
            f.treatment = src.reduce_mode;
            f.aux_p = src.aux_p;
            f.sw = ntt_switches();
            f.suppress_signal = e.ntt_suppress_signal;
            const FwdChoice c = select_fwd_half(f);
            if (!c.valid)
                return hipErrorInvalidValue;
            unsigned *tickets = c.tickets ? e.ntt_tickets(nrows) : nullptr;
            if (c.tickets && !tickets)
                return hipErrorOutOfMemory;
            NttSource ksrc = src;
            if (c.aux_as_doubles)
            {
                const double P = static_cast<double>(src.aux_p), Pinv = 1.0 / P;
                const double c0 = static_cast<double>(src.aux_top[0]), c2 = static_cast<double>(src.aux_top[2]);
                std::memcpy(&ksrc.aux_p, &P, 8);
                std::memcpy(&ksrc.aux_cr1, &Pinv, 8);
                std::memcpy(&ksrc.aux_top[0], &c0, 8);
                std::memcpy(&ksrc.aux_top[2], &c2, 8);
            }
            ProfScope prof(e, "ntt_fwd_half", transformed_rows(nrows, map));
            fwd_kernels<LOGN>()[c.instance]<<<static_cast<unsigned>(blocks), 1 << (LOGN - 6), lds_bytes, e.lane().stream>>>(
                data, e.d_primes, map, nrows, c.flags, tickets, e.lane().d_fault, e.ntt_spin_limit, ksrc, chunk, live);
            return hipGetLastError();
        }

        template <int LOGN>
        hipError_t init_half()
        {
            const int lds_bytes = hpad(1 << (LOGN - 2)) * 8;
            for (int i = 0; i < kFwdInstanceCount; i++)
                if (const FwdKernel k = fwd_kernels<LOGN>()[i])
                {
                    const hipError_t err = hipFuncSetAttribute(reinterpret_cast<const void *>(k), hipFuncAttributeMaxDynamicSharedMemorySize, lds_bytes);
                    if (err != hipSuccess)
                        return err;
                }
            return hipSuccess;
        }
    }

    hipError_t ntt_fwd_half(const Engine &e, u64 *data, std::size_t nrows, const RowMap &map, int flags, const NttSource &src)
    {
        switch (e.logn)
        {
        case 14: return launch_half<14>(e, data, nrows, map, flags, src);
        case 15: return launch_half<15>(e, data, nrows, map, flags, src);
        case 16: return launch_half<16>(e, data, nrows, map, flags, src);
        default: return hipErrorInvalidValue;
        }
    }

    hipError_t ntt_fwd_half_init()
    {
        hipError_t err = init_half<14>();
        if (err == hipSuccess)
            err = init_half<15>();
        if (err == hipSuccess)
            err = init_half<16>();
        return err;
    }
}
```

### gemini-seal_amd/csrc/ntt_half.hpp

```cpp
#pragma once
#include "engine.hpp"

#define SEALHIP_INTERNAL __attribute__((visibility("hidden")))

namespace sealhip
{
    SEALHIP_INTERNAL const NttSwitches &ntt_switches();
    SEALHIP_INTERNAL bool fp64_enabled();
    SEALHIP_INTERNAL bool exact_fwd();

    SEALHIP_INTERNAL hipError_t ntt_fwd_half(const Engine &e, u64 *data, std::size_t nrows, const RowMap &map, int flags,
                                             const NttSource &src);
    SEALHIP_INTERNAL hipError_t ntt_inv_half(const Engine &e, u64 *data, std::size_t nrows, const RowMap &map, int flags,
                                             const u64 *src = nullptr, std::size_t src_poly_stride = 0);
    SEALHIP_INTERNAL hipError_t ntt_inv_tensor(const Engine &e, u64 *data, std::size_t nrows, const RowMap &map, int flags,
                                               const u64 *x, std::size_t item_stride, std::size_t poly_stride, int kb,
                                               bool square);
    SEALHIP_INTERNAL hipError_t ntt_fwd_half_init();
    SEALHIP_INTERNAL hipError_t ntt_inv_half_init();

    namespace
    {
        template <int T, int R>
        struct Arr
        {
            static_assert(T >= 13 && T <= 15, "half-row shapes of N = 2^14 .. 2^16: 2^(T-5) lanes, i.e. 2^(T-11) waves <-> index bits [11, T)");
            static constexpr int beta = R <= 3 ? T - 4 * R : 0;
            static constexpr int f = T - 12;
            static constexpr int slot_bit(int w)
            {
                if (w == 0)
                    return 0;
                if (R <= 3)
                    return beta + (w - 1);
                if (w < f)
                    return w;
                return f + 6 + (w - f);
            }
            static constexpr int low_start = R <= 3 ? 1 : f;
            static constexpr int low_len = R <= 3 ? beta - 1 : T - 5;
            static constexpr int high_start = beta + 4;
            __device__ static __forceinline__ int tid_index(int tid)
            {
                if constexpr (R == 4)
                    return ((tid & 63) << f) | ((tid >> 6) << 11);
                int v = (tid & ((1 << low_len) - 1)) << low_start;
                if (R <= 3 && low_len < T - 5)
                    v |= (tid >> low_len) << high_start;
                return v;
            }
            static constexpr bool wave_owned = R == 2 || R == 3 || R == 4;
            static constexpr int slot_index(int s)
            {
                int r = 0;
                for (int w = 0; w < 5; w++)
                    if ((s >> w) & 1)
                        r |= 1 << slot_bit(w);
                return r;
            }
            static constexpr int tw_offset(int s, int w)
            {
                int r = 0;
                for (int v = w + 1; v < 5; v++)
                    if ((s >> v) & 1)
                        r |= 1 << (slot_bit(v) - slot_bit(w) - 1);
                return r;
            }
        };

        typedef u64 u64x2_nt __attribute__((ext_vector_type(2)));
        __device__ __forceinline__ void store_nt(u64 *p, u64 a, u64 b)
        {
            u64x2_nt v;
            v.x = a;
            v.y = b;
            __builtin_nontemporal_store(v, reinterpret_cast<u64x2_nt *>(p));
        }

        __host__ __device__ constexpr int hpad(int e)
        {
            return e + 2 * (e >> 5) + ((e >> 4) & 1);
        }

        template <int T, int RA, int RB>
        __device__ __forceinline__ void h_exchange(u64 (&x)[32], u64 *lds, int tid)
        {
            const int pa = hpad(Arr<T, RA>::tid_index(tid) >> 1);
            const int pb = hpad(Arr<T, RB>::tid_index(tid) >> 1);
            constexpr bool LOCAL = Arr<T, RA>::wave_owned && Arr<T, RB>::wave_owned;
            const auto sync = [] {
                if constexpr (LOCAL)
                {
                    __builtin_amdgcn_fence(__ATOMIC_RELEASE, "wavefront");
                    __builtin_amdgcn_wave_barrier();
                    __builtin_amdgcn_fence(__ATOMIC_ACQUIRE, "wavefront");
                }
                else
// ... 129 lines not shown
```

### gemini-seal_amd/csrc/ntt_select.hpp

```cpp
#pragma once
#include <cstdint>

#include "ntt_bounds.hpp"

namespace sealhip
{
    constexpr int kNttCanonical = 1;
    constexpr int kNttStrict = 2;
    constexpr int kNttAnyRep = 8;
    constexpr int kNttReduceOut = 0x10;
    constexpr int kNttApprox = 0x20;
    constexpr int kNttPolyMajor = 0x4000;
    constexpr int kNttSmallQuot = 0x1000000;
    constexpr int kNttDebugNoSignal = 0x40;
    constexpr int kNttTopDone = 0x80;
    constexpr int kNttDeferTop = 4;
    constexpr bounds::u64 kFpPrimeBound = bounds::u64(1) << bounds::kFpPrimeBits;

    constexpr int kSchedLazy = 0;
    constexpr int kSchedHarvey = 1;
    constexpr int kSchedApprox = 2;
    constexpr int kSchedFp64 = 3;
    constexpr int kSchedDense = 4;
    constexpr int kTreatNone = 0;
    constexpr int kTreatBarrett = 1;
    constexpr int kTreatCondSub = 2;
    constexpr int kTreatReduceOut = 3;
    constexpr int kTreatNegSpecial = 4;
    constexpr int kTreatNegSpecialTop = 5;
    constexpr int kTreatReduceOutTopDone = 6;
    constexpr int kTreatModDownStore = 7;
    constexpr int kInvExact = 0;
    constexpr int kInvLazySum = 1;
    constexpr int kInvFp64 = 2;
    constexpr int kInvDense = 3;
    constexpr int kShapeHalf = 0;
    constexpr int kShapeHalfTensor = 1;
    constexpr int kShapeWhole = 2;
    constexpr int kShapeQuarter = 3;
    constexpr int kTopNone = 0, kTopLayer = 1 , kTopRadix4 = 2 ;

    struct NttSwitches
    {
        bool no_fp64, exact_fwd, exact_inv, canon_exact;
    };

    struct FwdInstance
    {
        int sched, treatment;
    };
    constexpr FwdInstance kFwdInstances[] = {
        { kSchedLazy, kTreatNone },          { kSchedLazy, kTreatBarrett },        { kSchedLazy, kTreatCondSub },
        { kSchedLazy, kTreatReduceOut },     { kSchedLazy, kTreatNegSpecial },     { kSchedLazy, kTreatNegSpecialTop },
        { kSchedLazy, kTreatReduceOutTopDone },
        { kSchedHarvey, kTreatNone },        { kSchedHarvey, kTreatBarrett },      { kSchedHarvey, kTreatCondSub },
        { kSchedHarvey, kTreatReduceOut },   { kSchedHarvey, kTreatNegSpecial },   { kSchedHarvey, kTreatNegSpecialTop },
        { kSchedApprox, kTreatNone },        { kSchedApprox, kTreatBarrett },      { kSchedApprox, kTreatCondSub },
        { kSchedFp64, kTreatNone },          { kSchedFp64, kTreatBarrett },        { kSchedFp64, kTreatCondSub },
        { kSchedFp64, kTreatNegSpecial },    { kSchedFp64, kTreatNegSpecialTop },  { kSchedFp64, kTreatModDownStore },
        { kSchedDense, kTreatReduceOut },    { kSchedDense, kTreatReduceOutTopDone },
    };
    constexpr int kFwdInstanceCount = static_cast<int>(sizeof(kFwdInstances) / sizeof(kFwdInstances[0]));
    constexpr bool fwd_store_exchange(int T, int treatment)
    {
        return (T - 12) >= 2 && treatment == kTreatModDownStore;
    }
    constexpr bool fwd_instance_at(int logn, FwdInstance i)
    {
        return i.treatment != kTreatModDownStore || fwd_store_exchange(logn - 1, i.treatment);
    }
    constexpr int fwd_instance_index(int logn, int sched, int treatment)
    {
        for (int i = 0; i < kFwdInstanceCount; i++)
            if (kFwdInstances[i].sched == sched && kFwdInstances[i].treatment == treatment)
                return fwd_instance_at(logn, kFwdInstances[i]) ? i : -1;
        return -1;
    }

    struct InvInstance
    {
        int shape, sched;
        constexpr bool tensor_load() const
        {
            return shape == kShapeHalfTensor;
        }
    };
    constexpr InvInstance kInvInstances[] = {
        { kShapeHalf, kInvExact },       { kShapeHalf, kInvLazySum },       { kShapeHalf, kInvFp64 },    { kShapeHalf, kInvDense },
        { kShapeHalfTensor, kInvExact }, { kShapeHalfTensor, kInvLazySum }, { kShapeHalfTensor, kInvDense },
        { kShapeWhole, kInvExact },      { kShapeWhole, kInvLazySum },      { kShapeWhole, kInvFp64 },   { kShapeWhole, kInvDense },
        { kShapeQuarter, kInvExact },    { kShapeQuarter, kInvLazySum },    { kShapeQuarter, kInvFp64 }, { kShapeQuarter, kInvDense },
    };
    constexpr int kInvInstanceCount = static_cast<int>(sizeof(kInvInstances) / sizeof(kInvInstances[0]));
    constexpr bool inv_instance_at(int logn, InvInstance i)
    {
        return i.shape == kShapeWhole ? logn <= 15 : (i.shape == kShapeQuarter ? logn == 16 : true);
    }
    constexpr int inv_instance_index(int logn, int shape, int sched)
    {
        for (int i = 0; i < kInvInstanceCount; i++)
            if (kInvInstances[i].shape == shape && kInvInstances[i].sched == sched)
                return inv_instance_at(logn, kInvInstances[i]) ? i : -1;
        return -1;
    }
    constexpr int inv_kernel_logn(int shape, int logn)
    {
        return shape == kShapeWhole ? logn + 1 : (shape == kShapeQuarter ? logn - 1 : logn);
    }
    template <int KLOGN>
    constexpr int kInvLayers = KLOGN - 1;
    constexpr int inv_layers(int shape, int logn)
    {
        return inv_kernel_logn(shape, logn) - 1;
    }
    constexpr int inv_blocks_per_row(int shape)
    {
        return shape == kShapeWhole ? 1 : (shape == kShapeQuarter ? 4 : 2);
    }

    struct FwdFacts
    {
        int logn;
        int flags;
        const bounds::u64 *live;
        int live_n;
        bool gathers;
        bool all_gathered;
        bool same_source;
        int treatment;
        bounds::u64 aux_p;
        bool key_moduli_fp;
        NttSwitches sw;
        bool suppress_signal;
    };
    struct FwdChoice
    {
        bool valid;
        int instance;
        int sched, treatment;
        int flags;
        bool tickets;
        bool aux_as_doubles;
    };

    template <int LOGN>
    FwdChoice select_fwd_half_at(const FwdFacts &f)
    {
        FwdChoice c{};
        int flags = f.flags;
        const auto every_live = [&f](auto admits) {
            for (int i = 0; i < f.live_n; i++)
                if (!admits(f.live[i]))
                    return false;
            return true;
        };
        if ((flags & kNttStrict) != 0 && (flags & (kNttAnyRep | kNttCanonical | kNttApprox)) != 0 && (flags & kNttReduceOut) == 0)
        {
            if (!f.sw.exact_fwd && every_live([&](bounds::u64 p) { return bounds::fwd_canon_admits(p, LOGN); }))
                flags &= ~kNttStrict;
        }
        const bool dense = (flags & kNttStrict) != 0 && (flags & kNttReduceOut) != 0 && (flags & kNttAnyRep) != 0 &&
                           (flags & kNttCanonical) == 0 && !f.gathers && !f.sw.exact_fwd &&
                           every_live([&](bounds::u64 p) { return bounds::fwd_dense_admits(p, LOGN); });
        const bool top_done = (flags & kNttTopDone) != 0;
        if (top_done && (((flags & (kNttReduceOut | kNttStrict | kNttCanonical)) != kNttReduceOut && !dense) || f.gathers))
            return c;
        const bool all_gathered = f.gathers && f.all_gathered;
        c.tickets = !(top_done || all_gathered);
        if (f.suppress_signal)
            flags |= kNttDebugNoSignal;
        const bool one_source = all_gathered && f.treatment <= kTreatCondSub && f.live_n > 1 && f.same_source;
        bool fp = !f.sw.no_fp64 && (flags & (kNttAnyRep | kNttCanonical)) != 0 && (flags & kNttReduceOut) == 0 &&
                  every_live([](bounds::u64 p) { return p < kFpPrimeBound; });
        const bool special = f.treatment == kTreatNegSpecial || f.treatment == kTreatNegSpecialTop || f.treatment == kTreatModDownStore;
        if (fp && f.gathers)
        {
            if (special)
                fp = f.aux_p < (f.treatment == kTreatNegSpecial ? bounds::kFpInputBound : kFpPrimeBound);
            else
                fp = f.key_moduli_fp;
        }
        if (one_source && !fp)
        {
            const int g = 4 < f.live_n ? 4 : f.live_n;
            flags |= kNttPolyMajor | (g << 16);
        }
        if (flags & kNttAnyRep)
        {
            const bool ok = !f.sw.exact_fwd && (flags & (kNttCanonical | kNttStrict)) == 0 &&
                            every_live([&](bounds::u64 p) { return bounds::fwd_lazy_admits(p, LOGN); });
            if (!ok)
                flags &= ~kNttAnyRep;
        }
        int red = f.gathers ? f.treatment : kTreatNone;
        if (flags & kNttReduceOut)
        {
            if (red != kTreatNone || (flags & kNttCanonical))
                return c;
            red = top_done ? kTreatReduceOutTopDone : kTreatReduceOut;
        }
        const bool no_apx = f.sw.exact_fwd;
        bool apx = !no_apx && (flags & kNttApprox) != 0 && (flags & (kNttStrict | kNttCanonical | kNttReduceOut)) == 0 &&
                   !(f.gathers && special) && every_live([&](bounds::u64 p) { return bounds::fwd_lazy_admits(p, LOGN); });
        const bool capx = !no_apx && !f.sw.canon_exact && !fp && red == kTreatNone && (flags & kNttCanonical) != 0 &&
                          (flags & (kNttStrict | kNttReduceOut)) == 0 &&
                          every_live([&](bounds::u64 p) { return bounds::fwd_canon_admits(p, LOGN); });
        if (capx)
        {
            apx = true;
            flags |= kNttAnyRep;
            if (every_live([&](bounds::u64 p) { return bounds::small_quot_admits(p, bounds::fwd_canon_output_mult(LOGN)); }))
                flags |= kNttSmallQuot;
        }
        if (red == kTreatModDownStore && !fp)
            return c;
        c.sched = fp ? kSchedFp64 : (apx ? kSchedApprox : (dense ? kSchedDense : ((flags & kNttStrict) ? kSchedHarvey : kSchedLazy)));
        c.treatment = red;
        c.flags = flags;
        c.aux_as_doubles = fp && f.gathers && special;
        c.instance = fwd_instance_index(LOGN, c.sched, c.treatment);
        c.valid = c.instance >= 0;
        return c;
    }
    inline FwdChoice select_fwd_half(const FwdFacts &f)
    {
        switch (f.logn)
        {
        case 14: return select_fwd_half_at<14>(f);
        case 15: return select_fwd_half_at<15>(f);
        case 16: return select_fwd_half_at<16>(f);
        default: return FwdChoice{};
        }
    }

    struct InvFacts
    {
        int logn;
        int flags;
        const bounds::u64 *live;
        int live_n;
        bool tensor_load;
        NttSwitches sw;
    };
    struct InvChoice
    {
        bool valid;
        int instance;
        int shape, sched;
        int canon;
        int top;
    };

    template <int LAYERS>
    bool inv_lazy_all(const InvFacts &f)
    {
        for (int i = 0; i < f.live_n; i++)
            if (!bounds::inv_lazy_admits(LAYERS, f.live[i]))
                return false;
        return true;
    }
    template <int LAYERS>
    bool inv_dense_all(const InvFacts &f)
    {
        for (int i = 0; i < f.live_n; i++)
            if (!bounds::inv_dense_admits(LAYERS, f.live[i]))
                return false;
        return true;
    }

    template <int LOGN>
    InvChoice select_inv_half_at(const InvFacts &f)
    {
        InvChoice c{};
        const bool standalone = !f.tensor_load && !(f.flags & kNttDeferTop);
        c.shape = f.tensor_load ? kShapeHalfTensor : (!standalone ? kShapeHalf : (LOGN <= 15 ? kShapeWhole : kShapeQuarter));
        const bool any_rep = (f.flags & (kNttAnyRep | kNttCanonical)) != 0, lazy_ok = any_rep && !f.sw.exact_inv;
        bool lazy = lazy_ok && inv_lazy_all<kInvLayers<LOGN>>(f), dense = lazy_ok && inv_dense_all<kInvLayers<LOGN>>(f) && !lazy;
        if (c.shape == kShapeWhole)
        {
            constexpr int W = kInvLayers<inv_kernel_logn(kShapeWhole, LOGN)>;
            dense = (lazy || dense) && inv_dense_all<W>(f);
            lazy = lazy && inv_lazy_all<W>(f);
        }
        else if (c.shape == kShapeQuarter)
        {
            constexpr int Q = kInvLayers<inv_kernel_logn(kShapeQuarter, LOGN)>;
            lazy = lazy_ok && inv_lazy_all<Q>(f);
            dense = lazy_ok && inv_dense_all<Q>(f);
        }
        bool fp = any_rep && !f.sw.no_fp64 && !f.tensor_load;
        for (int i = 0; fp && i < f.live_n; i++)
            fp = f.live[i] < kFpPrimeBound;
        c.sched = fp ? kInvFp64 : (lazy ? kInvLazySum : (dense ? kInvDense : kInvExact));
        c.canon = (c.shape == kShapeWhole && (f.flags & kNttCanonical)) ? 1 : 0;
        c.top = c.shape == kShapeWhole ? kTopNone
                                       : (c.shape == kShapeQuarter ? kTopRadix4 : ((f.flags & kNttDeferTop) ? kTopNone : kTopLayer));
        c.instance = inv_instance_index(LOGN, c.shape, c.sched);
        c.valid = c.instance >= 0;
        return c;
    }
    inline InvChoice select_inv_half(const InvFacts &f)
    {
// ... 10 lines not shown
```

### gemini-seal_amd/csrc/pipeline.cpp

```cpp
#include "engine.hpp"

#include <cmath>

#include <algorithm>
#include <cstdlib>
#include <cstring>
#include <vector>

namespace sealhip
{
    namespace
    {
        std::size_t workspace_budget_bytes(const Engine &e)
        {
            Lane &l = e.lane();
            if (l.ws_budget)
                return l.ws_budget;
            static const std::size_t env_budget = [] {
                if (const char *env = std::getenv("SEALHIP_WORKSPACE_MB"))
                {
                    std::size_t mb = static_cast<std::size_t>(std::strtoull(env, nullptr, 10));
                    return (mb < 64 ? std::size_t(64) : mb) << 20;
                }
                return std::size_t(0);
// ... 69 lines not shown
    {
        const std::size_t chunk = plan_chunk(e, count, bytes_per_item, n_buffers);
        for (std::size_t off = 0; off < count; off += chunk)
        {
            e.ws_reset();
            body(off, std::min(chunk, count - off));
        }
    }

    RowMap ct_row_map(int rows, int polys, int only)
    {
        if (rows * polys > kMaxRows)
            throw std::invalid_argument("too many rows");
        RowMap m{};
        m.rows = rows * polys;
        for (int j = 0; j < polys; j++)
            for (int r = 0; r < rows; r++)
                m.prime[j * rows + r] = (only < 0 || only == j) ? static_cast<unsigned short>(r) : kSkipRow;
        return m;
    }

    namespace
    {
        struct KsArena
        {
            std::size_t w_coeff, w_ext, w_prod, w_temp;
            static constexpr int n_buffers = 4;
            std::size_t item_bytes() const
            {
                return (w_coeff + w_ext + w_prod + w_temp) * sizeof(u64);
            }
        };
        KsArena switch_key_arena(Engine &e, int k, bool rescale = false)
        {
            const std::size_t N = e.n, rows = static_cast<std::size_t>(k + e.nsp);
            const std::size_t nd = static_cast<std::size_t>(e.level(k).h_ks.nd);
            const bool has_coeff = e.scheme == 2 || e.mode_strict;
            return KsArena{ has_coeff ? static_cast<std::size_t>(k) * N : 0, nd * rows * N, 2 * rows * N,
                            2 * static_cast<std::size_t>(rescale ? k - 1 : k) * N };
        }

        unsigned *sink_at(Engine &e, std::size_t off)
        {
            Lane &l = e.lane();
            return l.tsink_cur ? l.tsink_cur + l.tsink_base + off : nullptr;
        }
        struct SinkArm
        {
            Lane &l;
            SinkArm(Engine &e, unsigned *flags) : l(e.lane())
            {
                l.tsink_arm = flags;
            }
            ~SinkArm()
            {
                l.tsink_arm = nullptr;
            }
        };
        struct FloorRestore
        {
            Lane &l;
            const std::size_t floor, base;
            explicit FloorRestore(Engine &e) : l(e.lane()), floor(l.ws_floor), base(l.tsink_base)
            {}
            ~FloorRestore()
            {
                l.ws_floor = floor;
                l.tsink_base = base;
            }
            void raise(std::size_t bytes)
            {
                l.ws_floor = floor + bytes;
            }
            void *parked() const
            {
                return static_cast<char *>(l.ws) + floor;
            }
        };

        struct KsRows
        {
            const u64 *inb;
            std::size_t inb_stride;
        };
        KsRows ks_digits(Engine &e, LevelTools &lt, int k, const u64 *tg, std::size_t target_stride, std::size_t m, u64 *coeff,
                         u64 *ext, int dj0, int dj1)
        {
            const KsDev &h = lt.h_ks;
            const std::size_t N = e.n;
            const int rows = k + e.nsp;
            const bool ckks = e.scheme == 2;
            const bool strict_bfv = e.mode_strict && !ckks;
            const RowMap map_q = lt.map_q;
            const RowMap map_rows = lt.map_key;
            const std::size_t ext_item = static_cast<std::size_t>(rows) * N;
            const std::size_t ext_digit = ext_item * m;
            const u64 *src = tg;
            std::size_t src_stride = target_stride;
            if (ckks)
            {
                if (ntt_can_gather(e))
                    check(launch_intt_from(e, coeff, tg, target_stride, m * k, map_q, kNttCanonical | kNttAnyRep),
                          "intt(target)");
                else
                {
                    check(launch_copy_rows(e, tg, target_stride, coeff, static_cast<std::size_t>(k) * N, m, k), "copy");
                    check(launch_ntt(e, coeff, m * k, map_q, true, kNttCanonical), "intt(target)");
                }
                src = coeff;
                src_stride = static_cast<std::size_t>(k) * N;
            }
            const bool gather = e.nsp == 1 && ntt_can_gather(e);
            bool need_any = false, need_barrett = false;
            for (int a = 0; a < k; a++)
                for (int b = 0; b < rows; b++)
                {
                    const u64 ps = e.key_moduli[h.row_prime[a]], pd = e.key_moduli[h.row_prime[b]];
                    need_any = need_any || (a != b && ps > pd);
                    need_barrett = need_barrett || (a != b && ps >= 2 * pd);
                }
            int modup_mode = need_barrett ? kTreatBarrett : (need_any ? kTreatCondSub : kTreatNone);
            if (modup_mode == kTreatCondSub)
            {
                u64 pmax = 0;
                for (int r = 0; r < rows; r++)
                    pmax = std::max(pmax, e.key_moduli[h.row_prime[r]]);
                if (bounds::fwd_lazy_admits(pmax, e.logn))
                    modup_mode = kTreatNone;
            }
            if (!gather)
                check(launch_ks_modup(e, lt.d_ks, h, src, src_stride, ext, ext_item, ext_digit, m, -1), "modup");
            for (int j = dj0; j < dj1; j++)
            {
                RowMap mj = map_rows;
                const int r0 = j * e.nsp, r1 = std::min(r0 + e.nsp, k);
                for (int r = r0; r < r1; r++)
                    mj.prime[r] = kSkipRow;
                if (gather)
                {
                    NttSource ns{};
                    ns.base[0] = src;
                    ns.poly_stride[0] = src_stride;
                    ns.reduce_mode = modup_mode;
                    const u64 p_src = e.key_moduli[h.row_prime[j]];
                    for (int r = 0; r < rows; r++)
                    {
                        if (r == j)
                        {
                            ns.code[r] = kSkipRow;
                            continue;
                        }
                        const u64 p_dst = e.key_moduli[h.row_prime[r]];
                        ns.code[r] = static_cast<unsigned short>(j | (p_src <= p_dst ? 0 : kSrcReduce));
                    }
                    check(launch_ntt_gather(e, ext + j * ext_digit, m * rows, mj, ns, kNttAnyRep | kNttApprox), "ntt(ext, gathered)");
                }
                else
                    check(launch_ntt(e, ext + j * ext_digit, m * rows, mj, false, kNttAnyRep), "ntt(ext)");
            }
            const u64 *inb = tg;
            std::size_t inb_stride = target_stride;
            if (strict_bfv)
            {
                if (ntt_can_gather(e))
                {
                    NttSource ns{};
                    ns.base[0] = tg;
                    ns.poly_stride[0] = target_stride;
                    for (int r = 0; r < k; r++)
                        ns.code[r] = static_cast<unsigned short>(r);
                    check(launch_ntt_gather(e, coeff, m * k, map_q, ns, kNttAnyRep | kNttApprox), "ntt(target, gathered)");
                }
                else
                {
                    check(launch_copy_rows(e, tg, target_stride, coeff, static_cast<std::size_t>(k) * N, m, k), "copy");
                    check(launch_ntt(e, coeff, m * k, map_q, false, 0), "ntt(target)");
                }
                inb = coeff;
                inb_stride = static_cast<std::size_t>(k) * N;
            }
            return KsRows{ inb, inb_stride };
        }

        void ks_products(Engine &e, LevelTools &lt, int k, const u64 *tg, std::size_t target_stride, std::size_t m, u64 *coeff,
                         u64 *ext, const KSwitchKey &key, u64 *prod, int dj0, int dj1)
        {
            const std::size_t ext_item = static_cast<std::size_t>(k + e.nsp) * e.n;
            const KsRows in_bundle = ks_digits(e, lt, k, tg, target_stride, m, coeff, ext, dj0, dj1);
            check(launch_ks_mac(e, lt.d_ks, lt.h_ks, in_bundle.inb, in_bundle.inb_stride, ext, ext_item, ext_item * m ,
                                key.d_data, prod, 2 * ext_item, m, dj0, dj1),
                  "mac");
        }

        void ks_finish(Engine &e, LevelTools &lt, int k, u64 *prod, u64 *temp, u64 *ctp, std::size_t ct_stride, const u64 *c0p,
                       std::size_t c0_stride, std::size_t m, unsigned *sink, bool one_component = false)
        {
            const KsDev &h = lt.h_ks;
            const std::size_t N = e.n;
            const int rows = k + e.nsp;
            const bool ckks = e.scheme == 2;
            const RowMap map_q = lt.map_q;
            const std::size_t ext_item = static_cast<std::size_t>(rows) * N;
            RowMap map_rows = lt.map_key;
            u64 *const prod_rows = one_component ? prod - ext_item : prod;
            const std::size_t npolys = one_component ? m : 2 * m, prod_stride = one_component ? 2 * ext_item : ext_item;
            const int lead = one_component ? rows : 0;
            if (one_component)
            {
                if (c0p || sink || ct_stride != 2 * static_cast<std::size_t>(k) * N || 2 * rows > kMaxRows)
                    throw std::logic_error("internal: one-component mod-down misused");
                map_rows.rows = 2 * rows;
                for (int r = 0; r < rows; r++)
                {
                    map_rows.prime[rows + r] = map_rows.prime[r];
                    map_rows.prime[r] = kSkipRow;
                }
            }
            if (!ckks)
            {
                const bool defer = ntt_can_defer_top(e, k);
                check(launch_ntt(e, prod_rows, m * 2 * rows, map_rows, true, (defer ? kNttDeferTop : 0) | kNttAnyRep), "intt(prod)");
                SinkArm arm(e, sink);
                check(launch_ks_moddown_bfv(e, lt.d_ks, h, prod, prod_stride, ctp, ct_stride, npolys, defer, c0p, c0_stride),
                      "moddown_bfv");
                return;
            }
            const u64 p_special = (ckks && e.nsp == 1) ? e.key_moduli[h.row_prime[k]] : 0;
            bool fold_ok = ckks && e.nsp == 1 && ntt_can_gather(e);
            for (int r = 0; fold_ok && r < k; r++)
            {
                const u64 q = e.key_moduli[h.row_prime[r]];
                fold_ok = p_special <= q || (p_special < 2 * q && bounds::fwd_lazy_admits(q, e.logn));
            }
            const bool fold_pre = fold_ok;
            const bool fold_top = fold_pre && ntt_can_defer_top(e, k);
            const bool fold_store = fold_top && ntt_can_fuse_moddown(e, k, p_special);
            check(launch_ntt(e, prod_rows, m * 2 * rows, skip_map(map_rows, lead + k, lead + rows), true,
                             kNttAnyRep | (fold_top ? kNttDeferTop : 0)),
                  "intt(special)");
            if (fold_pre)
            {
                NttSource ns{};
                ns.base[0] = prod;
                ns.poly_stride[0] = prod_stride;
                ns.reduce_mode = fold_store ? kTreatModDownStore : (fold_top ? kTreatNegSpecialTop : kTreatNegSpecial);
                if (fold_store)
                {
                    ns.md.inv_p = lt.d_ks->invP;
                    ns.md.inv_p_shoup = lt.d_ks->invP_shoup;
                    ns.md.prod = prod;
                    ns.md.prod_stride = prod_stride;
                    ns.md.ct = ctp;
                    ns.md.ct_stride = ct_stride;
                    ns.md.c0_src = c0p;
                    ns.md.c0_stride = c0_stride;
                    ns.md.tflags = sink;
                }
                ns.aux_p = p_special;
                ns.aux_cr1 = HostModulus(p_special).cr1;
                {
                    const HostNttTables &tb = e.tables[h.row_prime[k]];
                    ns.aux_top[0] = tb.inv_n;
                    ns.aux_top[1] = tb.inv_n_shoup;
                    ns.aux_top[2] = tb.inv_n_w;
                    ns.aux_top[3] = tb.inv_n_w_shoup;
                }
                for (int r = 0; r < k; r++)
                    ns.code[r] = static_cast<unsigned short>(k);
                check(launch_ntt_gather(e, temp, npolys * k, map_q, ns, kNttAnyRep), "ntt(temp, gathered from the special row)");
            }
            else
            {
                check(launch_ks_moddown_pre(e, lt.d_ks, h, prod, prod_stride, temp, static_cast<std::size_t>(k) * N, npolys),
                      "moddown_pre");
                if (ckks)
                    check(launch_ntt(e, temp, npolys * k, map_q, false, kNttAnyRep), "ntt(temp)");
                else
                    check(launch_ntt(e, prod_rows, m * 2 * rows, skip_map(map_rows, lead, lead + k), true, kNttAnyRep), "intt(prod)");
            }
            if (!fold_store)
            {
                SinkArm arm(e, sink);
                check(launch_ks_moddown_post(e, lt.d_ks, h, prod, prod_stride, temp, static_cast<std::size_t>(k) * N, ctp,
                                             ct_stride, npolys, 1, c0p, c0_stride),
                      "moddown_post");
            }
        }

        void ks_finish_rescale(Engine &e, LevelTools &lt, int k, const u64 *base, std::size_t base_stride, u64 *acc, u64 *temp,
                               u64 *out, std::size_t m, unsigned *sink)
        {
            if (e.scheme != 2 || k < 2 || !lt.d_ksr)
                throw std::logic_error("internal: merged rescale misused");
            const KsRescaleDev &h = lt.h_ksr;
            const std::size_t N = e.n;
            const int rows = k + e.nsp;
            const std::size_t ext_item = static_cast<std::size_t>(rows) * N;
            check(launch_ks_rescale_fold(e, lt.d_ksr, h, base, base_stride, acc, ext_item, 2 * m), "rescale_fold");
            check(launch_ntt(e, acc, m * 2 * rows, skip_map(lt.map_key, k - 1, rows), true, kNttCanonical), "intt(dropped)");
            check(launch_ks_moddown_rescale_pre(e, lt.d_ksr, h, acc, ext_item, temp, 2 * m), "moddown_rescale_pre");
            check(launch_ntt(e, temp, m * 2 * (k - 1), e.level_host(k - 1).map_q, false, kNttCanonical | kNttStrict), "ntt(temp)");
            SinkArm arm(e, sink);
            check(launch_ks_moddown_rescale_post(e, lt.d_ksr, h, base, base_stride, acc, ext_item, temp, out, 2 * m),
                  "moddown_rescale_post");
        }
    }

    void op_switch_key(Engine &e, int k, u64 *ct, std::size_t ct_stride, const u64 *target, std::size_t target_stride,
                       std::size_t count, const KSwitchKey &key, const u64 *c0_src, std::size_t c0_stride, const KsSplit *split)
    {
        if (k > e.k_first)
            throw std::invalid_argument("key switching needs a ciphertext level");
        LevelTools &lt = e.level(k);
        const KsDev &h = lt.h_ks;
        const bool finish = split && split->partial_sum;
        const bool partial = split && split->partial_out;
        if (!finish && (static_cast<int>(key.n_digits) < h.nd || (key.level && k > static_cast<int>(key.level))))
            throw std::invalid_argument("kswitch_keys is not valid for encryption parameters");
        const int dj0 = partial ? split->j0 : 0, dj1 = partial ? split->j1 : h.nd;
        if (dj0 < 0 || dj0 > dj1 || dj1 > h.nd)
            throw std::invalid_argument("digit range out of bounds");
        const int rows = k + e.nsp;
        const KsArena ar = switch_key_arena(e, k);
        const RowMap map_rows = lt.map_key;
        for_chunks(e, count, ar.item_bytes(), KsArena::n_buffers, [&](std::size_t off, std::size_t m) {
            u64 *coeff = ar.w_coeff ? e.ws_alloc(ar.w_coeff * m) : nullptr;
            u64 *ext = e.ws_alloc(ar.w_ext * m);
            u64 *prod = e.ws_alloc(ar.w_prod * m);
            u64 *temp = e.ws_alloc(ar.w_temp * m);
            if (partial)
                prod = split->partial_out + off * ar.w_prod;
            if (finish)
                prod = split->partial_sum + off * ar.w_prod;
            u64 *ctp = partial ? nullptr : ct + off * ct_stride;
            const u64 *c0p = c0_src ? c0_src + off * c0_stride : nullptr;

            if (finish)
                check(launch_poly_op(e, PolyOp::Mod63, prod, nullptr, 0, prod, m * 2 * rows, map_rows), "mod(partial sum)");
            else
                ks_products(e, lt, k, target + off * target_stride, target_stride, m, coeff, ext, key, prod, dj0, dj1);
            if (partial)
                return;
            ks_finish(e, lt, k, prod, temp, ctp, ct_stride, c0p, c0_stride, m, sink_at(e, off));
        });
    }

    void op_switch_secret(Engine &e, int k, const u64 *c0, const u64 *c1, std::size_t stride, std::size_t count,
                          const KSwitchKey &key, u64 *out)
    {
        op_switch_key(e, k, out, 2 * static_cast<std::size_t>(k) * e.n, c1, stride, count, key, c0, stride);
    }

    void op_switch_key_rescale(Engine &e, int k, const u64 *base, std::size_t base_stride, const u64 *target,
                               std::size_t target_stride, std::size_t count, const KSwitchKey &key, u64 *out)
    {
        if (e.scheme != 2)
            throw std::invalid_argument("the merged rescale is a CKKS operation");
        if (k > e.k_first)
            throw std::invalid_argument("key switching needs a ciphertext level");
        if (k < 2)
            throw std::invalid_argument("end of modulus switching chain reached");
        LevelTools &lt = e.level_rescale(k);
        const KsDev &h = lt.h_ks;
        if (static_cast<int>(key.n_digits) < h.nd)
            throw std::invalid_argument("kswitch_keys is not valid for encryption parameters");
        const KsArena ar = switch_key_arena(e, k, true);
        for_chunks(e, count, ar.item_bytes(), KsArena::n_buffers, [&](std::size_t off, std::size_t m) {
            u64 *coeff = e.ws_alloc(ar.w_coeff * m);
            u64 *ext = e.ws_alloc(ar.w_ext * m);
            u64 *prod = e.ws_alloc(ar.w_prod * m);
            u64 *temp = e.ws_alloc(ar.w_temp * m);
            ks_products(e, lt, k, target + off * target_stride, target_stride, m, coeff, ext, key, prod, 0, h.nd);
            ks_finish_rescale(e, lt, k, base + off * base_stride, base_stride, prod, temp, out + off * ar.w_temp, m,
                              sink_at(e, off));
        });
    }

    void op_double_angle(Engine &e, int k, const u64 *ct, std::size_t count, const u64 *constant, const KSwitchKey &key, u64 *out)
    {
        if (e.scheme != 2)
            throw std::invalid_argument("the merged rescale is a CKKS operation");
        if (k > e.k_first)
            throw std::invalid_argument("key switching needs a ciphertext level");
        if (k < 2)
            throw std::invalid_argument("end of modulus switching chain reached");
        LevelTools &lt = e.level_rescale(k);
        if (static_cast<int>(key.n_digits) < lt.h_ks.nd)
            throw std::invalid_argument("kswitch_keys is not valid for encryption parameters");
// ... 1448 lines not shown
```

### gemini-seal_amd/sealhip/__init__.py

```python
import ctypes as C
import os

import numpy as np

_HERE = os.path.dirname(os.path.abspath(__file__))
LIB_PATH = os.environ.get("SEALHIP_LIBRARY") or os.path.join(os.path.dirname(_HERE), "lib", "libsealhip.so")

S_OK = 0
E_POINTER = 0x80004003
E_INVALIDARG = 0x80070057
E_OUTOFMEMORY = 0x8007000E
E_UNEXPECTED = 0x8000FFFF
COR_E_INVALIDOPERATION = 0x80131509

SCHEME_BFV, SCHEME_CKKS = 1, 2
MODE_PARITY, MODE_STRICT = 0, 1
BASE_Q, BASE_BSK, BASE_KEY = 0, 1, 2


class LogicError(RuntimeError):
    """std::logic_error of the reference (unsupported operation for the scheme, host-only context, ...)."""


class Params(C.Structure):
    _fields_ = [
        ("scheme", C.c_uint32),
        ("log_n", C.c_uint32),
        ("n_key_moduli", C.c_uint32),
        ("n_special_primes", C.c_uint32),
        ("key_moduli", C.POINTER(C.c_uint64)),
        ("plain_modulus", C.c_uint64),
        ("mode", C.c_uint32),
        ("device", C.c_int32),
    ]


_lib = None

_vp, _u32, _u64, _sz, _i32 = C.c_void_p, C.c_uint32, C.c_uint64, C.c_size_t, C.c_int32


class PolyPlan(C.Structure):
    _fields_ = [("d", _u32), ("m", _u32), ("g", _u32), ("inner_level", _u32), ("out_level", _u32), ("n_products", _u32),
                ("out_scale", C.c_double), ("temp_bytes_per_item", _u64)]


class DftStage(C.Structure):
    _fields_ = [("s0", _u32), ("r", _u32), ("h0", _u32), ("level", _u32), ("n_baby", _u32), ("n_giant", _u32), ("folded", _u32),
                ("reserved", _u32), ("scale", C.c_double)]


class DftPlan(C.Structure):
    _fields_ = [("direction", _u32), ("n_stages", _u32), ("in_level", _u32), ("out_level", _u32), ("needs_conjugation", _u32),
                ("n_key_steps", _u32), ("table_words", _u64), ("temp_bytes_per_item", _u64), ("stages", DftStage * 16)]


class EvalModPlan(C.Structure):
    _fields_ = [("K", _u32), ("r", _u32), ("degree", _u32), ("n_baby", _u32), ("poly_level", _u32), ("out_level", _u32),
                ("n_products", _u32), ("reserved", _u32), ("poly_scale_out", C.c_double), ("scales", C.c_double * 9),
                ("temp_bytes_per_item", _u64)]


class BootstrapPlan(C.Structure):
    _fields_ = [("k_top", _u32), ("c2s_out_level", _u32), ("evalmod_out_level", _u32), ("out_level", _u32),
                ("needs_conjugation", _u32), ("n_key_steps", _u32), ("raise_scale", C.c_double), ("s2c_gain", C.c_double),
                ("table_words", _u64), ("temp_bytes_per_item", _u64), ("evalmod", EvalModPlan)]


DFT_COEFFS_TO_SLOTS, DFT_SLOTS_TO_COEFFS = 0, 1

SYMBOLS = {
    "sealhip_last_error_string": None,
    "sealhip_num_devices": [C.POINTER(C.c_int32)],
    "sealhip_context_create": [C.POINTER(Params), C.POINTER(_vp)],
    "sealhip_context_destroy": [_vp],
    "sealhip_context_first_level": [_vp, C.POINTER(_u32)],
    "sealhip_context_bsk_size": [_vp, _u32, C.POINTER(_u32)],
    "sealhip_set_stream": [_vp, _vp],
    "sealhip_use_default_stream": [_vp],
    "sealhip_synchronize": [_vp],
    "sealhip_context_lane_count": [_vp, C.POINTER(_u32)],
    "sealhip_debug_ntt_handoff": [_vp, _u32, _i32],
    "sealhip_malloc": [_vp, _sz, C.POINTER(_vp)],
    "sealhip_free": [_vp, _vp],
    "sealhip_memcpy_h2d": [_vp, _vp, _vp, _sz],
    "sealhip_memcpy_d2h": [_vp, _vp, _vp, _sz],
    "sealhip_profile_enable": [_vp, _i32],
    "sealhip_profile_fetch": [_vp, C.c_char_p, _sz],
    "sealhip_debug_ntt_table": [_vp, _u32, _u32, _vp, _sz],
    "sealhip_debug_rns_constants": [_vp, _u32, _u32, _vp, _sz, C.POINTER(_sz)],
    "sealhip_debug_bfv_multiply_plan": [_vp, _u32, _u32, _u32, _i32, _vp],
    "sealhip_debug_behz_dot_split": [_vp, _u32, C.POINTER(C.c_int32)],
    "sealhip_ntt_negacyclic_harvey_lazy": [_vp, _vp, _sz, _u32, _u32],
    "sealhip_ntt_negacyclic_harvey": [_vp, _vp, _sz, _u32, _u32],
    "sealhip_inverse_ntt_negacyclic_harvey_lazy": [_vp, _vp, _sz, _u32, _u32],
    "sealhip_inverse_ntt_negacyclic_harvey": [_vp, _vp, _sz, _u32, _u32],
    "sealhip_dyadic_product_coeffmod": [_vp, _vp, _vp, _sz, _u32, _u32, _vp],
    "sealhip_multiply_poly_scalar_coeffmod": [_vp, _vp, _sz, _u32, _u32, _u64, _vp],
    "sealhip_add_poly_coeffmod": [_vp, _vp, _vp, _sz, _u32, _u32, _vp],
    "sealhip_sub_poly_coeffmod": [_vp, _vp, _vp, _sz, _u32, _u32, _vp],
    "sealhip_negate_poly_coeffmod": [_vp, _vp, _sz, _u32, _u32, _vp],
    "sealhip_fastbconv_m_tilde": [_vp, _u32, _vp, _sz, _vp],
    "sealhip_sm_mrq": [_vp, _u32, _vp, _sz, _vp],
    "sealhip_fast_floor": [_vp, _u32, _vp, _sz, _vp],
    "sealhip_fastbconv_sk": [_vp, _u32, _vp, _sz, _vp],
    "sealhip_divide_and_round_q_last_inplace": [_vp, _u32, _vp, _sz],
    "sealhip_divide_and_round_q_last_ntt_inplace": [_vp, _u32, _vp, _sz],
    "sealhip_galois_elt_from_step": [_vp, _i32, C.POINTER(_u32)],
    "sealhip_apply_galois": [_vp, _vp, _sz, _u32, _u32, _vp],
    "sealhip_apply_galois_ntt": [_vp, _vp, _sz, _u32, _u32, _vp],
    "sealhip_kswitch_key_load": [_vp, _vp, _u32, _i32, C.POINTER(_vp)],
    "sealhip_kswitch_key_destroy": [_vp, _vp],
    "sealhip_modup_rns": [_vp, _u32, _u32, _vp, _sz],
    "sealhip_rescale_special_rns_inplace": [_vp, _u32, _vp, _sz],
    "sealhip_switch_key_inplace": [_vp, _u32, _vp, _vp, _sz, _vp],
    "sealhip_switch_key_partial": [_vp, _u32, _vp, _sz, _vp, _u32, _u32, _vp],
    "sealhip_switch_key_finish": [_vp, _u32, _vp, _vp, _sz, _u32],
    "sealhip_kswitch_digits": [_vp, _u32, _vp],
    "sealhip_evaluator_multiply": [_vp, _u32, _vp, _u32, _vp, _u32, _sz, _vp],
    "sealhip_evaluator_square": [_vp, _u32, _vp, _u32, _sz, _vp],
    "sealhip_evaluator_relinearize": [_vp, _u32, _vp, _u32, _sz, C.POINTER(_vp), _u32],
    "sealhip_evaluator_multiply_many": [_vp, _u32, _vp, _u32, _sz, C.POINTER(_vp), _u32, _vp],
    "sealhip_evaluator_exponentiate": [_vp, _u32, _vp, _u64, _sz, C.POINTER(_vp), _u32, _vp],
    "sealhip_evaluator_multiply_host": [_vp, _u32, _vp, _u32, _vp, _u32, _sz, _vp, C.POINTER(_vp), _u32],
    "sealhip_evaluator_relinearize_host": [_vp, _u32, _vp, _u32, _sz, C.POINTER(_vp), _u32],
    "sealhip_evaluator_rotate_vector_host": [_vp, _u32, _vp, _sz, _i32, C.POINTER(_u32), C.POINTER(_vp), _u32],
    "sealhip_evaluator_mod_switch_to_next_host": [_vp, _u32, _vp, _u32, _sz, _vp],
    "sealhip_evaluator_rescale_to_next_host": [_vp, _u32, _vp, _u32, _sz, _vp],
    "sealhip_evaluator_mod_switch_to_next": [_vp, _u32, _vp, _u32, _sz, _vp],
    "sealhip_evaluator_rescale_to_next": [_vp, _u32, _vp, _u32, _sz, _vp],
    "sealhip_evaluator_mod_switch_to_next_strided": [_vp, _u32, _vp, _u32, _sz, _sz, _vp],
    "sealhip_evaluator_rescale_to_next_strided": [_vp, _u32, _vp, _u32, _sz, _sz, _vp],
    "sealhip_evaluator_apply_galois": [_vp, _u32, _vp, _sz, _u32, _vp],
    "sealhip_evaluator_transform_to_ntt": [_vp, _u32, _vp, _u32, _sz],
    "sealhip_evaluator_transform_from_ntt": [_vp, _u32, _vp, _u32, _sz],
    "sealhip_evaluator_negate": [_vp, _u32, _vp, _u32, _sz, _vp],
    "sealhip_evaluator_add": [_vp, _u32, _vp, _u32, _vp, _u32, _sz, _vp],
    "sealhip_evaluator_sub": [_vp, _u32, _vp, _u32, _vp, _u32, _sz, _vp],
    "sealhip_evaluator_multiply_plain_ntt": [_vp, _u32, _vp, _u32, _sz, _vp, _sz],
    "sealhip_evaluator_multiply_plain": [_vp, _u32, _vp, _u32, _sz, _vp, _sz],
    "sealhip_evaluator_transform_plain_to_ntt": [_vp, _u32, _vp, _sz, _sz, _sz, _vp],
    "sealhip_evaluator_mod_switch_plain_to": [_vp, _u32, _vp, _sz, _u32, _vp],
    "sealhip_is_transparent": [_vp, _u32, _vp, _u32, _sz, _vp],
    "sealhip_transparency_sink": [_vp, _vp, _sz],
    "sealhip_debug_butterfly_rate": [_vp, _u32, _u32, _vp],
    "sealhip_debug_chunk_log": [_vp, _vp, _sz, _vp],
    "sealhip_modulo_poly_coeffs_63": [_vp, _vp, _sz, _u32, _u32, _vp],
    "sealhip_evaluator_rotate_vector": [_vp, _u32, _vp, _sz, _i32, C.POINTER(_u32), C.POINTER(_vp), _u32],
    "sealhip_evaluator_apply_galois_many": [_vp, _u32, _vp, _sz, C.POINTER(_u32), C.POINTER(_vp), _u32, _vp],
    "sealhip_evaluator_rotate_vector_many": [_vp, _u32, _vp, _sz, C.POINTER(_i32), _u32, C.POINTER(_u32), C.POINTER(_vp), _u32,
                                             _vp],
    "sealhip_evaluator_apply_galois_dot_plain": [_vp, _u32, _vp, _sz, C.POINTER(_u32), C.POINTER(_vp), _u32, _vp, _u32, _vp],
    "sealhip_evaluator_rotate_vector_dot_plain": [_vp, _u32, _vp, _sz, C.POINTER(_i32), _u32, C.POINTER(_u32), C.POINTER(_vp),
                                                  _u32, _vp, _u32, _vp],
    "sealhip_evaluator_apply_galois_bsgs_plain": [_vp, _u32, _vp, _sz, C.POINTER(_u32), C.POINTER(_vp), _u32, C.POINTER(_u32),
                                                  C.POINTER(_vp), _u32, _vp, _vp],
    "sealhip_evaluator_rotate_vector_bsgs_plain": [_vp, _u32, _vp, _sz, C.POINTER(_i32), _u32, C.POINTER(_i32), _u32,
                                                   C.POINTER(_u32), C.POINTER(_vp), _u32, _vp, _vp],
    "sealhip_evaluator_dot_product_max_terms": [_vp, _u32, C.POINTER(C.c_uint64)],
    "sealhip_evaluator_dot_product": [_vp, _u32, C.POINTER(_vp), C.POINTER(_vp), _u32, _sz, C.POINTER(_vp), _u32, _vp],
    "sealhip_evaluator_linear_combination": [_vp, _u32, C.POINTER(_vp), _u32, _u32, _sz, _vp, _vp, _u32, _vp],
    "sealhip_evaluator_polynomial_plan_ckks": [_vp, _u32, C.c_double, C.POINTER(C.c_double), _u32, _u32, _u32, C.c_double, _vp,
                                               C.POINTER(_u64), C.POINTER(_u64)],
    "sealhip_evaluator_evaluate_polynomial_ckks": [_vp, _u32, _vp, _sz, C.c_double, C.POINTER(C.c_double), _u32, _u32, _u32,
                                                   C.c_double, C.POINTER(_vp), _u32, _vp, C.POINTER(_u32),
                                                   C.POINTER(C.c_double)],
    "sealhip_evaluator_linear_combination_levels": [_vp, _u32, C.POINTER(_vp), C.POINTER(_u32), C.POINTER(_u32), _u32, _u32, _sz,
                                                    _vp, _vp, _u32, _vp],
    "sealhip_evaluator_evaluate_polynomial": [_vp, _u32, _vp, _sz, C.POINTER(C.c_uint64), _u32, _u32, C.POINTER(_vp), _u32, _vp],
    "sealhip_evaluator_relinearize_rescale": [_vp, _u32, _vp, _u32, _sz, _sz, C.POINTER(_vp), _u32, _vp],
    "sealhip_evaluator_dot_product_rescale": [_vp, _u32, C.POINTER(_vp), C.POINTER(_vp), _u32, _sz, C.POINTER(_vp), _u32, _vp],
    "sealhip_evaluator_apply_galois_dot_plain_rescale": [_vp, _u32, _vp, _sz, C.POINTER(_u32), C.POINTER(_vp), _u32, _vp, _u32,
                                                         _vp],
    "sealhip_evaluator_rotate_vector_dot_plain_rescale": [_vp, _u32, _vp, _sz, C.POINTER(_i32), _u32, C.POINTER(_u32),
                                                          C.POINTER(_vp), _u32, _vp, _u32, _vp],
# ... 308 lines not shown
    def synchronize(self):
        _check(lib().sealhip_synchronize(self.handle))

    def pool_alloc(self, words):
        return PoolBuffer(self, words)

    def pool_release(self, ptr):
        _check(lib().sealhip_pool_release(self.handle, _ptr(ptr)))

    def pool_trim(self):
        _check(lib().sealhip_pool_trim(self.handle))

    def pool_stats(self):
        st = PoolStats()
        _check(lib().sealhip_pool_stats(self.handle, C.byref(st)))
        return {name: int(getattr(st, name)) for name, _ in PoolStats._fields_}

    def memcpy_d2d(self, dst, src, words):
        _check(lib().sealhip_memcpy_d2d(self.handle, _ptr(dst), _ptr(src), int(words) * 8))

    def transparency_note(self, k, ct, size, count):
        _check(lib().sealhip_transparency_note(self.handle, k, _ptr(ct), size, count))

    def set_stream(self, stream_ptr):
        _check(lib().sealhip_set_stream(self.handle, stream_ptr))

    def lane_count(self):
        v = C.c_uint32()
        _check(lib().sealhip_context_lane_count(self.handle, C.byref(v)))
        return v.value

    def use_default_stream(self):
        _check(lib().sealhip_use_default_stream(self.handle))

    def debug_ntt_handoff(self, spin_limit=0, suppress_signal=False):
        _check(lib().sealhip_debug_ntt_handoff(self.handle, spin_limit, 1 if suppress_signal else 0))

    def bsk_size(self, k):
        v = C.c_uint32()
        _check(lib().sealhip_context_bsk_size(self.handle, k, C.byref(v)))
        return v.value

    def rows(self, k, base):
        if base == BASE_Q:
            return k
        if base == BASE_BSK:
            return self.bsk_size(k)
        return k + self.nsp

    def profile_enable(self, on=True):
        _check(lib().sealhip_profile_enable(self.handle, 1 if on else 0))

    def profile_fetch(self):
        import json

        buf = C.create_string_buffer(1 << 16)
        _check(lib().sealhip_profile_fetch(self.handle, buf, len(buf)))
        return json.loads(buf.value.decode())

    def debug_ntt_table(self, prime_index, kind):
        out = np.empty(self.n, dtype=np.uint64)
        _check(lib().sealhip_debug_ntt_table(self.handle, prime_index, kind, out.ctypes.data, out.size))
        return out

    def debug_rns_constants(self, k, which):
        out = np.empty(70 * 70, dtype=np.uint64)
        w = C.c_size_t()
        _check(lib().sealhip_debug_rns_constants(self.handle, k, which, out.ctypes.data, out.size, C.byref(w)))
        return out[: w.value].copy()

    BFV_PLAN_FIELDS = ("k", "B", "nB", "square", "redc_small", "gather", "defer", "fused_tensor", "tensor_apx", "lift_top",
                       "lift_kernel", "floor_kernel", "deferred_top")

    def debug_bfv_multiply_plan(self, k, size_a=2, size_b=2, square=False):
        out = np.zeros(len(self.BFV_PLAN_FIELDS), dtype=np.int32)
        _check(lib().sealhip_debug_bfv_multiply_plan(self.handle, k, size_a, size_b, 1 if square else 0, out.ctypes.data))
        return dict(zip(self.BFV_PLAN_FIELDS, (int(x) for x in out)))

    def debug_behz_dot_split(self, k):
        v = C.c_int32()
        _check(lib().sealhip_debug_behz_dot_split(self.handle, k, C.byref(v)))
        return v.value

    def galois_elt_from_step(self, step):
        v = C.c_uint32()
        _check(lib().sealhip_galois_elt_from_step(self.handle, step, C.byref(v)))
        return v.value

    def ntt_negacyclic_harvey_lazy(self, data, count, k, base=BASE_Q):
        _check(lib().sealhip_ntt_negacyclic_harvey_lazy(self.handle, _ptr(data), count, k, base))

    def ntt_negacyclic_harvey(self, data, count, k, base=BASE_Q):
        _check(lib().sealhip_ntt_negacyclic_harvey(self.handle, _ptr(data), count, k, base))

    def inverse_ntt_negacyclic_harvey_lazy(self, data, count, k, base=BASE_Q):
        _check(lib().sealhip_inverse_ntt_negacyclic_harvey_lazy(self.handle, _ptr(data), count, k, base))

    def inverse_ntt_negacyclic_harvey(self, data, count, k, base=BASE_Q):
        _check(lib().sealhip_inverse_ntt_negacyclic_harvey(self.handle, _ptr(data), count, k, base))

    def dyadic_product_coeffmod(self, a, b, count, k, result, base=BASE_Q):
        _check(lib().sealhip_dyadic_product_coeffmod(self.handle, _ptr(a), _ptr(b), count, k, base, _ptr(result)))

    def multiply_poly_scalar_coeffmod(self, a, count, k, scalar, result, base=BASE_Q):
        _check(lib().sealhip_multiply_poly_scalar_coeffmod(self.handle, _ptr(a), count, k, base, scalar, _ptr(result)))

    def add_poly_coeffmod(self, a, b, count, k, result, base=BASE_Q):
        _check(lib().sealhip_add_poly_coeffmod(self.handle, _ptr(a), _ptr(b), count, k, base, _ptr(result)))

    def sub_poly_coeffmod(self, a, b, count, k, result, base=BASE_Q):
        _check(lib().sealhip_sub_poly_coeffmod(self.handle, _ptr(a), _ptr(b), count, k, base, _ptr(result)))

    def modulo_poly_coeffs_63(self, a, count, k, result, base=BASE_Q):
        _check(lib().sealhip_modulo_poly_coeffs_63(self.handle, _ptr(a), count, k, base, _ptr(result)))

    def is_transparent(self, ct, size, k, count):
        flags = np.zeros(count, dtype=np.uint8)
        _check(lib().sealhip_is_transparent(self.handle, k, _ptr(ct), size, count, flags.ctypes.data))
        return flags.astype(bool)

    def transparency_sink(self, flags, capacity):
        _check(lib().sealhip_transparency_sink(self.handle, _ptr(flags) if flags is not None else None, capacity))

    def dot_product_ct_sk(self, ct, size, k, count, sk_powers_ntt, is_ntt_form, out):
        _check(lib().sealhip_decryptor_dot_product_ct_sk(self.handle, k, _ptr(ct), size, count, _ptr(sk_powers_ntt),
                                                         1 if is_ntt_form else 0, _ptr(out)))

    def decrypt_scale_and_round(self, k, poly, count, out):
        _check(lib().sealhip_decrypt_scale_and_round(self.handle, k, _ptr(poly), count, _ptr(out)))

    def invariant_noise_budget(self, ct, size, k, count, sk_powers_ntt):
        budgets = np.zeros(max(1, count), dtype=np.int32)
        _check(lib().sealhip_decryptor_invariant_noise_budget(self.handle, k, _ptr(ct), size, count, _ptr(sk_powers_ntt),
                                                              budgets.ctypes.data))
        return budgets[:count]

    def decrypt(self, ct, size, k, count, sk_powers_ntt, is_ntt_form, plain):
        _check(lib().sealhip_decryptor_decrypt(self.handle, k, _ptr(ct), size, count, _ptr(sk_powers_ntt),
                                               1 if is_ntt_form else 0, _ptr(plain)))

    def encrypt_zero_symmetric(self, rows, is_ntt_form, a_ntt, noise, sk_ntt, count, ct):
        _check(lib().sealhip_encrypt_zero_symmetric(self.handle, rows, 1 if is_ntt_form else 0, _ptr(a_ntt), _ptr(noise),
                                                    _ptr(sk_ntt), count, _ptr(ct)))

    def encrypt(self, k, pk_ntt, plain, u, noise, count, ct, plain_item_stride=None):
        if plain_item_stride is None:
            plain_item_stride = self.n if self.scheme == SCHEME_BFV else k * self.n
        _check(lib().sealhip_encryptor_encrypt(self.handle, k, _ptr(pk_ntt), _ptr(plain) if plain is not None else None,
                                               plain_item_stride, _ptr(u), _ptr(noise), count, _ptr(ct)))

    def encrypt_symmetric(self, k, sk_ntt, plain, seeds, noise, count, ct, save_seed=False, plain_item_stride=None):
        if plain_item_stride is None:
            plain_item_stride = self.n if self.scheme == SCHEME_BFV else k * self.n
        seeds = np.ascontiguousarray(np.asarray(seeds, dtype=np.uint64).reshape(-1))
        _check(lib().sealhip_encryptor_encrypt_symmetric(self.handle, k, _ptr(sk_ntt),
                                                         _ptr(plain) if plain is not None else None, plain_item_stride,
                                                         seeds.ctypes.data, _ptr(noise), 1 if save_seed else 0, count,
                                                         _ptr(ct)))

    def save_seeded(self, info, src, seed_words):
        seed = np.ascontiguousarray(np.array([int(x) for x in seed_words], dtype=np.uint64))
        need = _sz(0)
        _check(lib().sealhip_ciphertext_save_seeded(self.handle, C.addressof(info), _ptr(src), seed.ctypes.data, None, 0,
                                                    C.byref(need)))
        buf = (C.c_char * need.value)()
        written = _sz(0)
# ... 799 lines not shown
```

### include/sealhip.h

```cpp
#ifndef SEALHIP_H
#define SEALHIP_H

#include <stddef.h>
#include <stdint.h>

#ifdef __cplusplus
extern "C" {
#endif

#define SEALHIP_S_OK 0L
#define SEALHIP_E_POINTER ((long)0x80004003L)
#define SEALHIP_E_INVALIDARG ((long)0x80070057L)
#define SEALHIP_E_OUTOFMEMORY ((long)0x8007000EL)
#define SEALHIP_E_UNEXPECTED ((long)0x8000FFFFL)
#define SEALHIP_COR_E_INVALIDOPERATION ((long)0x80131509L)

#define SEALHIP_SCHEME_BFV 1u
#define SEALHIP_SCHEME_CKKS 2u

#define SEALHIP_MODE_PARITY 0u
#define SEALHIP_MODE_STRICT 1u

#define SEALHIP_BASE_Q 0u
#define SEALHIP_BASE_BSK 1u
#define SEALHIP_BASE_KEY 2u

typedef struct sealhip_context sealhip_context;
typedef struct sealhip_kswitch_key sealhip_kswitch_key;

typedef struct sealhip_params
{
    uint32_t scheme;
    uint32_t log_n;
    uint32_t n_key_moduli;
    uint32_t n_special_primes;
    const uint64_t *key_moduli;
    uint64_t plain_modulus;
    uint32_t mode;
    int32_t device;
} sealhip_params;

const char *sealhip_last_error_string(void);
long sealhip_num_devices(int32_t *count);
long sealhip_context_create(const sealhip_params *params, sealhip_context **out);
long sealhip_context_destroy(sealhip_context *ctx);
long sealhip_context_first_level(const sealhip_context *ctx, uint32_t *k_first);
long sealhip_context_bsk_size(sealhip_context *ctx, uint32_t k, uint32_t *bsk_size);
long sealhip_set_stream(sealhip_context *ctx, void *hip_stream);
long sealhip_use_default_stream(sealhip_context *ctx);
long sealhip_synchronize(sealhip_context *ctx);
long sealhip_context_lane_count(sealhip_context *ctx, uint32_t *lanes);

long sealhip_malloc(sealhip_context *ctx, size_t bytes, void **dptr);
long sealhip_free(sealhip_context *ctx, void *dptr);
long sealhip_memcpy_h2d(sealhip_context *ctx, void *dst_dev, const void *src_host, size_t bytes);
long sealhip_memcpy_d2h(sealhip_context *ctx, void *dst_host, const void *src_dev, size_t bytes);

struct sealhip_pool_stats
{
    uint64_t bytes_in_use;
    uint64_t bytes_cached;
    uint64_t device_mallocs;
    uint64_t device_frees;
    uint64_t hits;
    uint64_t misses;
    uint64_t cross_lane_hits;
};
long sealhip_pool_alloc(sealhip_context *ctx, size_t bytes, void **dptr);
long sealhip_pool_release(sealhip_context *ctx, void *dptr);
long sealhip_pool_trim(sealhip_context *ctx);
long sealhip_pool_stats(sealhip_context *ctx, struct sealhip_pool_stats *out);
long sealhip_memcpy_d2d(sealhip_context *ctx, void *dst_dev, const void *src_dev, size_t bytes);
long sealhip_transparency_note(sealhip_context *ctx, uint32_t k, const uint64_t *ct, uint32_t size, size_t count);

long sealhip_profile_enable(sealhip_context *ctx, int32_t enable);
long sealhip_profile_fetch(sealhip_context *ctx, char *json, size_t capacity);

long sealhip_debug_ntt_handoff(sealhip_context *ctx, uint32_t spin_limit, int32_t suppress_signal);

long sealhip_debug_chunk_log(sealhip_context *ctx, size_t *count_chunk_pairs, size_t capacity_pairs, size_t *written);

long sealhip_debug_butterfly_rate(sealhip_context *ctx, uint32_t kind, uint32_t prime_index, double *butterflies_per_s);

long sealhip_debug_ntt_table(sealhip_context *ctx, uint32_t prime_index, uint32_t kind, uint64_t *out_host,
                             size_t capacity);
long sealhip_debug_rns_constants(sealhip_context *ctx, uint32_t k, uint32_t which, uint64_t *out_host,
                                 size_t capacity, size_t *written);
long sealhip_debug_bfv_multiply_plan(sealhip_context *ctx, uint32_t k, uint32_t size_a, uint32_t size_b, int32_t square,
                                     int32_t *out);
long sealhip_debug_behz_dot_split(sealhip_context *ctx, uint32_t k, int32_t *out);

long sealhip_ntt_negacyclic_harvey_lazy(sealhip_context *ctx, uint64_t *data, size_t count, uint32_t k,
                                        uint32_t base);
long sealhip_ntt_negacyclic_harvey(sealhip_context *ctx, uint64_t *data, size_t count, uint32_t k, uint32_t base);
long sealhip_inverse_ntt_negacyclic_harvey_lazy(sealhip_context *ctx, uint64_t *data, size_t count, uint32_t k,
                                                uint32_t base);
long sealhip_inverse_ntt_negacyclic_harvey(sealhip_context *ctx, uint64_t *data, size_t count, uint32_t k,
                                           uint32_t base);

long sealhip_dyadic_product_coeffmod(sealhip_context *ctx, const uint64_t *a, const uint64_t *b, size_t count,
                                     uint32_t k, uint32_t base, uint64_t *result);
long sealhip_multiply_poly_scalar_coeffmod(sealhip_context *ctx, const uint64_t *a, size_t count, uint32_t k,
                                           uint32_t base, uint64_t scalar, uint64_t *result);
long sealhip_add_poly_coeffmod(sealhip_context *ctx, const uint64_t *a, const uint64_t *b, size_t count, uint32_t k,
                               uint32_t base, uint64_t *result);
long sealhip_sub_poly_coeffmod(sealhip_context *ctx, const uint64_t *a, const uint64_t *b, size_t count, uint32_t k,
                               uint32_t base, uint64_t *result);
long sealhip_negate_poly_coeffmod(sealhip_context *ctx, const uint64_t *a, size_t count, uint32_t k, uint32_t base,
                                  uint64_t *result);

long sealhip_fastbconv_m_tilde(sealhip_context *ctx, uint32_t k, const uint64_t *in, size_t count, uint64_t *out);
long sealhip_sm_mrq(sealhip_context *ctx, uint32_t k, const uint64_t *in, size_t count, uint64_t *out);
long sealhip_fast_floor(sealhip_context *ctx, uint32_t k, const uint64_t *in, size_t count, uint64_t *out);
long sealhip_fastbconv_sk(sealhip_context *ctx, uint32_t k, const uint64_t *in, size_t count, uint64_t *out);
long sealhip_divide_and_round_q_last_inplace(sealhip_context *ctx, uint32_t k, uint64_t *data, size_t count);
long sealhip_divide_and_round_q_last_ntt_inplace(sealhip_context *ctx, uint32_t k, uint64_t *data, size_t count);

long sealhip_galois_elt_from_step(const sealhip_context *ctx, int32_t step, uint32_t *galois_elt);
long sealhip_apply_galois(sealhip_context *ctx, const uint64_t *in, size_t count, uint32_t k, uint32_t galois_elt,
                          uint64_t *out);
long sealhip_apply_galois_ntt(sealhip_context *ctx, const uint64_t *in, size_t count, uint32_t k,
                              uint32_t galois_elt, uint64_t *out);

long sealhip_kswitch_key_load(sealhip_context *ctx, const uint64_t *key, uint32_t n_digits, int32_t from_host,
                              sealhip_kswitch_key **out);
long sealhip_kswitch_key_destroy(sealhip_context *ctx, sealhip_kswitch_key *key);
long sealhip_modup_rns(sealhip_context *ctx, uint32_t k, uint32_t src_bundle_index, uint64_t *ext, size_t count);
long sealhip_rescale_special_rns_inplace(sealhip_context *ctx, uint32_t k, uint64_t *poly, size_t count);
long sealhip_switch_key_inplace(sealhip_context *ctx, uint32_t k, uint64_t *ct, const uint64_t *target, size_t count,
                                const sealhip_kswitch_key *key);
long sealhip_switch_key_partial(sealhip_context *ctx, uint32_t k, const uint64_t *target, size_t count,
                                const sealhip_kswitch_key *key, uint32_t digit_begin, uint32_t digit_end, uint64_t *partial);
long sealhip_switch_key_finish(sealhip_context *ctx, uint32_t k, uint64_t *ct, uint64_t *partial_sum, size_t count,
                               uint32_t n_partials);
long sealhip_kswitch_digits(sealhip_context *ctx, uint32_t k, uint32_t *digits);

long sealhip_evaluator_multiply(sealhip_context *ctx, uint32_t k, const uint64_t *a, uint32_t size_a,
                                const uint64_t *b, uint32_t size_b, size_t count, uint64_t *out);
long sealhip_evaluator_square(sealhip_context *ctx, uint32_t k, const uint64_t *a, uint32_t size_a, size_t count,
                              uint64_t *out);
long sealhip_evaluator_relinearize(sealhip_context *ctx, uint32_t k, uint64_t *ct, uint32_t size, size_t count,
                                   const sealhip_kswitch_key *const *relin_keys, uint32_t n_relin_keys);
long sealhip_evaluator_mod_switch_to_next(sealhip_context *ctx, uint32_t k, const uint64_t *ct, uint32_t size,
                                          size_t count, uint64_t *out);
long sealhip_evaluator_rescale_to_next(sealhip_context *ctx, uint32_t k, const uint64_t *ct, uint32_t size,
                                       size_t count, uint64_t *out);
long sealhip_evaluator_mod_switch_to_next_strided(sealhip_context *ctx, uint32_t k, const uint64_t *ct, uint32_t size,
                                                  size_t ct_item_stride, size_t count, uint64_t *out);
long sealhip_evaluator_rescale_to_next_strided(sealhip_context *ctx, uint32_t k, const uint64_t *ct, uint32_t size,
                                               size_t ct_item_stride, size_t count, uint64_t *out);
long sealhip_evaluator_apply_galois(sealhip_context *ctx, uint32_t k, uint64_t *ct, size_t count,
                                    uint32_t galois_elt, const sealhip_kswitch_key *galois_key);
long sealhip_evaluator_transform_to_ntt(sealhip_context *ctx, uint32_t k, uint64_t *ct, uint32_t size, size_t count);
long sealhip_evaluator_transform_from_ntt(sealhip_context *ctx, uint32_t k, uint64_t *ct, uint32_t size,
                                          size_t count);

long sealhip_evaluator_multiply_many(sealhip_context *ctx, uint32_t k, const uint64_t *const *encrypteds, uint32_t n_encrypteds,
                                     size_t count, const sealhip_kswitch_key *const *relin_keys, uint32_t n_relin_keys,
                                     uint64_t *out);
long sealhip_evaluator_exponentiate(sealhip_context *ctx, uint32_t k, const uint64_t *ct, uint64_t exponent, size_t count,
                                    const sealhip_kswitch_key *const *relin_keys, uint32_t n_relin_keys, uint64_t *out);

long sealhip_evaluator_multiply_host(sealhip_context *ctx, uint32_t k, const uint64_t *const *a, uint32_t size_a,
                                     const uint64_t *const *b, uint32_t size_b, size_t count, uint64_t *const *out,
                                     const sealhip_kswitch_key *const *relin_keys, uint32_t n_relin_keys);
long sealhip_evaluator_relinearize_host(sealhip_context *ctx, uint32_t k, uint64_t *const *ct, uint32_t size, size_t count,
                                        const sealhip_kswitch_key *const *relin_keys, uint32_t n_relin_keys);
long sealhip_evaluator_rotate_vector_host(sealhip_context *ctx, uint32_t k, uint64_t *const *ct, size_t count, int32_t steps,
                                          const uint32_t *galois_elts, const sealhip_kswitch_key *const *galois_keys,
                                          uint32_t n_keys);
long sealhip_evaluator_mod_switch_to_next_host(sealhip_context *ctx, uint32_t k, const uint64_t *const *ct, uint32_t size,
                                               size_t count, uint64_t *const *out);
long sealhip_evaluator_rescale_to_next_host(sealhip_context *ctx, uint32_t k, const uint64_t *const *ct, uint32_t size,
// ... 327 lines not shown
```

Before: 24330.

## Fuse last forward NTT stage of key-switch digits into paired MAC kernel

```diff
diff --git a/gemini-seal_amd/csrc/api.cpp b/gemini-seal_amd/csrc/api.cpp
--- a/gemini-seal_amd/csrc/api.cpp
+++ b/gemini-seal_amd/csrc/api.cpp
@@ -729,6 +729,41 @@
     });
 }
 
+long sealhip_debug_ks_split_last(sealhip_context *ctx, uint32_t k, size_t count, int32_t *out)
+{
+    REQUIRE_PTR(ctx);
+    REQUIRE_PTR(out);
+    return guarded([&] {
+        Engine &e = device_engine(ctx);
+        check_level(e, k);
+        *out = ks_split_last_plan(e, static_cast<int>(k), count) ? 1 : 0;
+    });
+}
+
+long sealhip_debug_ntt_split_last(sealhip_context *ctx, uint32_t prime_index, uint32_t treatment, int32_t exact,
+                                  const uint64_t *src_device, uint64_t *dst_device)
+{
+    REQUIRE_PTR(ctx);
+    REQUIRE_PTR(src_device);
+    REQUIRE_PTR(dst_device);
+    return guarded([&] {
+        Engine &e = device_engine(ctx);
+        if (prime_index >= e.key_moduli.size() || treatment > 2 || src_device == dst_device)
+            throw std::invalid_argument("ntt_split_last: a key prime, treatment 0..2, distinct buffers");
+        RowMap map{};
+        map.rows = 1;
+        map.prime[0] = static_cast<unsigned short>(prime_index);
+        NttSource ns{};
+        ns.base[0] = reinterpret_cast<const u64 *>(src_device);
+        ns.code[0] = 0;
+        ns.reduce_mode = static_cast<int>(treatment);
+        const int flags = exact ? 0 : (kNttAnyRep | kNttApprox);
+        if (!ntt_can_split_last(e, map, ns, flags, 1))
+            throw std::invalid_argument("ntt_split_last: no instance of this form for the ring and prime");
+        SEALHIP_CHECK(launch_ntt_gather(e, reinterpret_cast<u64 *>(dst_device), 1, map, ns, flags | kNttSplitLast));
+    });
+}
+
 long sealhip_debug_behz_dot_split(sealhip_context *ctx, uint32_t k, int32_t *out)
 {
     REQUIRE_PTR(ctx);
diff --git a/gemini-seal_amd/csrc/engine.hpp b/gemini-seal_amd/csrc/engine.hpp
--- a/gemini-seal_amd/csrc/engine.hpp
+++ b/gemini-seal_amd/csrc/engine.hpp
@@ -386,6 +386,7 @@
     bool ntt_strict_top_done_ok(const Engine &e, const RowMap &map);
     hipError_t launch_ntt_gather(const Engine &e, u64 *data, std::size_t nrows, const RowMap &map, const NttSource &src,
                                  int flags);
+    bool ntt_can_split_last(const Engine &e, const RowMap &map, const NttSource &src, int flags, int nd);
 
     enum class PolyOp
     {
@@ -461,6 +462,7 @@
         int deferred_top;
     };
     BfvMulPlan plan_bfv_multiply(Engine &e, int k, int sa, int sb, bool square);
+    bool ks_split_last_plan(Engine &e, int k, std::size_t count);
 
     bool bfv_lift_can_apply_top(const Engine &e, int k, bool redc_small);
     hipError_t launch_bfv_lift(const Engine &e, const RnsDev *d, const RnsDev &h, const u64 *in, std::size_t in_stride,
@@ -557,7 +559,9 @@
     hipError_t launch_ks_mac(const Engine &e, const KsDev *d, const KsDev &h, const u64 *target,
                              std::size_t target_stride, const u64 *ext, std::size_t ext_stride,
                              std::size_t ext_digit_stride, const u64 *key, u64 *prod, std::size_t prod_stride,
-                             std::size_t count, int j0 = 0, int j1 = -1);
+                             std::size_t count, int j0 = 0, int j1 = -1,
+                             bool pair = false);
+    bool ks_mac_has_pair_form(const Engine &e, const KsDev &h, std::size_t count, int j0, int j1);
     hipError_t launch_ks_moddown_pre(const Engine &e, const KsDev *d, const KsDev &h, const u64 *prod,
                                      std::size_t prod_stride, u64 *temp, std::size_t temp_stride, std::size_t npolys);
     hipError_t launch_ks_moddown_bfv(const Engine &e, const KsDev *d, const KsDev &h, const u64 *prod,
diff --git a/gemini-seal_amd/csrc/keyswitch.hip b/gemini-seal_amd/csrc/keyswitch.hip
--- a/gemini-seal_amd/csrc/keyswitch.hip
+++ b/gemini-seal_amd/csrc/keyswitch.hip
@@ -191,6 +191,122 @@
             }
         }
 
+        __device__ __forceinline__ void mac128_wide(u64 &lo, u64 &hi, u64 a, u64 b)
+        {
+            const unsigned __int128 acc = ((static_cast<unsigned __int128>(hi) << 64) | lo) + static_cast<unsigned __int128>(a) * b;
+            lo = static_cast<u64>(acc);
+            hi = static_cast<u64>(acc >> 64);
+        }
+
+        template <int ND, bool PF>
+        __global__ __launch_bounds__(kThreads) void ks_mac_pair_kernel(const KsDev *__restrict__ d,
+                                                                       const PrimeDev *__restrict__ primes,
+                                                                       const u64 *__restrict__ target,
+                                                                       std::size_t target_stride,
+                                                                       const u64 *__restrict__ ext, std::size_t ext_stride,
+                                                                       std::size_t ext_digit_stride,
+                                                                       const u64 *__restrict__ key,
+                                                                       u64 *__restrict__ prod, std::size_t prod_stride,
+                                                                       std::size_t count, int logn, std::size_t group)
+        {
+            const std::size_t N = static_cast<std::size_t>(1) << logn, H = N >> 1;
+            const int k = d->k, nsp = d->nsp, rows = k + nsp, n_total = d->n_total;
+            const std::size_t lane0 = blockIdx.x * static_cast<std::size_t>(kThreads);
+            const std::size_t c0 = lane0 & (H - 1);
+            const std::size_t rr = lane0 >> (logn - 1);
+            const int r = static_cast<int>(rr % rows);
+            const std::size_t item0 = (rr / rows) * group;
+            if (item0 >= count)
+                return;
+            const std::size_t item1 = item0 + group < count ? item0 + group : count;
+            const int rns_idx = d->row_prime[r];
+            const int my_digit = r < k ? r / nsp : -1;
+            const std::size_t row_off = static_cast<std::size_t>(r) * N;
+            const PrimeDev &P = primes[rns_idx];
+            const u64 p = P.p, two_p = P.two_p, cr0 = P.cr0, cr1 = P.cr1;
+            const unsigned off8 = threadIdx.x * 8u, off16 = threadIdx.x * 16u;
+            const auto word = [](const u64 *base, unsigned off) {
+                return *reinterpret_cast<const u64 *>(reinterpret_cast<const char *>(base) + off);
+            };
+            const auto pair = [](const u64 *base, unsigned off) {
+                return *reinterpret_cast<const ulonglong2 *>(reinterpret_cast<const char *>(base) + off);
+            };
+            const u64 *key_row = key + static_cast<std::size_t>(rns_idx) * N + 2 * c0;
+            const std::size_t key_comp = static_cast<std::size_t>(n_total) * N;
+            const ulonglong2 w = pair(P.fwd + 2 * (H + c0), off16);
+            ulonglong2 k0[ND], k1[ND];
+#pragma unroll
+            for (int j = 0; j < ND; j++)
+            {
+                k0[j] = pair(key_row + (2 * static_cast<std::size_t>(j)) * key_comp, off16);
+                k1[j] = pair(key_row + (2 * static_cast<std::size_t>(j) + 1) * key_comp, off16);
+            }
+            const u64 *src[ND];
+#pragma unroll
+            for (int j = 0; j < ND; j++)
+                src[j] = j == my_digit ? target + item0 * target_stride + row_off + 2 * c0
+                                       : ext + item0 * ext_stride + static_cast<std::size_t>(j) * ext_digit_stride + row_off + c0;
+            const unsigned off8_o = off8 + (static_cast<unsigned>(H) << 3), off16_o = off16 + 8u;
+            const auto load_x = [&](u64(&e)[ND], u64(&o)[ND]) {
+#pragma unroll
+                for (int j = 0; j < ND; j++)
+                {
+                    const bool inb = j == my_digit;
+                    e[j] = word(src[j], inb ? off16 : off8);
+                    o[j] = word(src[j], inb ? off16_o : off8_o);
+                    src[j] += inb ? target_stride : ext_stride;
+                }
+            };
+            const auto accumulate = [&](const u64(&e)[ND], const u64(&o)[ND], std::size_t item) {
+                u64 lo00 = 0, hi00 = 0, lo01 = 0, hi01 = 0, lo10 = 0, hi10 = 0, lo11 = 0, hi11 = 0;
+#pragma unroll
+                for (int j = 0; j < ND; j++)
+                {
+                    u64 x0 = e[j], x1 = o[j];
+                    if (j != my_digit)
+                    {
+                        const u64 t = mulmod_lazy(x1, w.x, w.y, p);
+                        x1 = x0 - t + two_p;
+                        x0 = x0 + t;
+                    }
+                    mac128_wide(lo00, hi00, x0, k0[j].x);
+                    mac128_wide(lo01, hi01, x1, k0[j].y);
+                    mac128_wide(lo10, hi10, x0, k1[j].x);
+                    mac128_wide(lo11, hi11, x1, k1[j].y);
+                }
+                u64 *pp = reinterpret_cast<u64 *>(reinterpret_cast<char *>(prod + item * prod_stride + row_off + 2 * c0) + off16);
+                store_stream2(pp, barrett_reduce_128(lo00, hi00, p, cr0, cr1), barrett_reduce_128(lo01, hi01, p, cr0, cr1));
+                store_stream2(pp + static_cast<std::size_t>(rows) * N, barrett_reduce_128(lo10, hi10, p, cr0, cr1),
+                              barrett_reduce_128(lo11, hi11, p, cr0, cr1));
+            };
+            u64 xe[ND], xo[ND];
+            load_x(xe, xo);
+            if constexpr (PF)
+            {
+                u64 ne[ND], no[ND];
+                for (std::size_t item = item0; item < item1; item += 2)
+                {
+                    if (item + 1 < item1)
+                        load_x(ne, no);
+                    accumulate(xe, xo, item);
+                    if (item + 1 >= item1)
+                        break;
+                    if (item + 2 < item1)
+                        load_x(xe, xo);
+                    accumulate(ne, no, item + 1);
+                }
+            }
+            else
+                for (std::size_t item = item0; item < item1; item++)
+                {
+                    accumulate(xe, xo, item);
+                    if (item + 1 < item1)
+                        load_x(xe, xo);
+                }
+        }
+
+        constexpr int kKsPairPrefetchDigits = 8;
+
         __global__ __launch_bounds__(kThreads) void ks_moddown_pre_kernel(const KsDev *__restrict__ d,
                                                                           const PrimeDev *__restrict__ primes,
                                                                           const u64 *__restrict__ prod,
@@ -501,10 +617,15 @@
         return hipGetLastError();
     }
 
+    bool ks_mac_has_pair_form(const Engine &e, const KsDev &h, std::size_t count, int j0, int j1)
+    {
+        return e.logn >= 14 && count >= 16 && j0 == 0 && j1 == h.nd && h.nd >= 1 && h.nd <= 16;
+    }
+
     hipError_t launch_ks_mac(const Engine &e, const KsDev *d, const KsDev &h, const u64 *target,
                              std::size_t target_stride, const u64 *ext, std::size_t ext_stride,
                              std::size_t ext_digit_stride, const u64 *key, u64 *prod, std::size_t prod_stride,
-                             std::size_t count, int j0, int j1)
+                             std::size_t count, int j0, int j1, bool pair)
     {
         if (!count)
             return hipSuccess;
@@ -513,6 +634,8 @@
         if (j0 < 0 || j0 > j1 || j1 > h.nd)
             return hipErrorInvalidValue;
         const bool all_digits = j0 == 0 && j1 == h.nd;
+        if (pair && !ks_mac_has_pair_form(e, h, count, j0, j1))
+            return hipErrorInvalidValue;
         const u64 *tg = target;
         const std::size_t lanes = (count * static_cast<std::size_t>(h.k + h.nsp)) << e.logn;
         ProfScope prof(e, "ks_mac", 0);
@@ -527,6 +650,37 @@
             }
         const std::size_t groups = (count + mac_group - 1) / mac_group;
         const std::size_t glanes = (groups * static_cast<std::size_t>(h.k + h.nsp)) << e.logn;
+        if (pair)
+        {
+            const std::size_t planes = (groups * static_cast<std::size_t>(h.k + h.nsp)) << (e.logn - 1);
+#define SEALHIP_KS_MAC_PAIR(ND)                                                                                                          \
+    case ND:                                                                                                                             \
+        ks_mac_pair_kernel<ND, (ND <= kKsPairPrefetchDigits)><<<blocks_for(planes), kThreads, 0, e.lane().stream>>>(                    \
+            d, e.d_primes, tg, target_stride, ext, ext_stride, ext_digit_stride, key, prod, prod_stride, count, e.logn, mac_group); \
+        break;
+            switch (h.nd)
+            {
+                SEALHIP_KS_MAC_PAIR(1)
+                SEALHIP_KS_MAC_PAIR(2)
+                SEALHIP_KS_MAC_PAIR(3)
+                SEALHIP_KS_MAC_PAIR(4)
+                SEALHIP_KS_MAC_PAIR(5)
+                SEALHIP_KS_MAC_PAIR(6)
+                SEALHIP_KS_MAC_PAIR(7)
+                SEALHIP_KS_MAC_PAIR(8)
+                SEALHIP_KS_MAC_PAIR(9)
+                SEALHIP_KS_MAC_PAIR(10)
+                SEALHIP_KS_MAC_PAIR(11)
+                SEALHIP_KS_MAC_PAIR(12)
+                SEALHIP_KS_MAC_PAIR(13)
+                SEALHIP_KS_MAC_PAIR(14)
+                SEALHIP_KS_MAC_PAIR(15)
+                SEALHIP_KS_MAC_PAIR(16)
+            default: return hipErrorInvalidValue;
+            }
+#undef SEALHIP_KS_MAC_PAIR
+            return hipGetLastError();
+        }
 #define SEALHIP_KS_MAC(ND)                                                                                          \
     case ND:                                                                                                        \
         ks_mac_items_kernel<ND><<<blocks_for(glanes), kThreads, 0, e.lane().stream>>>(                                     \
diff --git a/gemini-seal_amd/csrc/ntt.hip b/gemini-seal_amd/csrc/ntt.hip
--- a/gemini-seal_amd/csrc/ntt.hip
+++ b/gemini-seal_amd/csrc/ntt.hip
@@ -527,6 +527,16 @@
         return e.use_half_kernel && e.logn >= 14 && e.logn <= 16;
     }
 
+    bool ntt_can_split_last(const Engine &e, const RowMap &map, const NttSource &src, int flags, int nd)
+    {
+        if (!ntt_can_gather(e))
+            return false;
+        for (int r = 0; r < map.rows; r++)
+            if (map.prime[r] != kSkipRow && !bounds::fwd_split_admits(e.tables[map.prime[r]].p, e.logn, nd))
+                return false;
+        return ntt_fwd_half_splits(e, map, flags | (e.mode_strict ? kNttStrict : 0), src);
+    }
+
     hipError_t launch_ntt_gather(const Engine &e, u64 *data, size_t nrows, const RowMap &map, const NttSource &src,
                                  int flags)
     {
diff --git a/gemini-seal_amd/csrc/ntt_bounds.hpp b/gemini-seal_amd/csrc/ntt_bounds.hpp
--- a/gemini-seal_amd/csrc/ntt_bounds.hpp
+++ b/gemini-seal_amd/csrc/ntt_bounds.hpp
@@ -167,6 +167,30 @@
         }
         static_assert(fwd_dense_peak_mult(14) == 14 && fwd_dense_peak_mult(15) == 14 && fwd_dense_peak_mult(16) == 16,
                       "dense forward schedule: 14p after round 1, at most 16p after the final round at N = 2^16");
+
+        constexpr int fwd_split_output_mult(int logn)
+        {
+            return 2 + kFwdApxGrowth * (logn - 1);
+        }
+        constexpr u128 fwd_split_peak(int logn, u64 p)
+        {
+            return fwd_int_peak(logn - 1, p, 2, true, true) + static_cast<u128>(2) * p;
+        }
+        constexpr int fwd_split_prime_bits(int logn)
+        {
+            int bits = 0;
+            for (int b = 1; b <= kMaxPrimeBits; b++)
+                if (fwd_split_peak(logn, max_prime_of_bits(b)) < kWord)
+                    bits = b;
+            return bits;
+        }
+        static_assert(kFwdApxLevel != 2 || (fwd_split_prime_bits(14) == 58 && fwd_split_prime_bits(15) == 58 && fwd_split_prime_bits(16) == 58),
+                      "split form at level 2: 56p / 60p / 64p at log n = 14 / 15 / 16, below 2^64 for primes below 2^58");
+        constexpr bool fwd_split_admits(u64 p, int logn, int nd)
+        {
+            return logn >= kMinHalfLogn && logn <= kMaxHalfLogn && nd >= 1 && p <= max_prime_of_bits(fwd_split_prime_bits(logn)) &&
+                   static_cast<u128>(nd) * p < kWord;
+        }
 
         constexpr bool tensor_redc_ok(u64 p, int operand_mult, int np)
         {
diff --git a/gemini-seal_amd/csrc/ntt_fwd.hip b/gemini-seal_amd/csrc/ntt_fwd.hip
--- a/gemini-seal_amd/csrc/ntt_fwd.hip
+++ b/gemini-seal_amd/csrc/ntt_fwd.hip
@@ -568,6 +568,44 @@
             }
         }
 
+        template <int T, int HALF, int REDUCE>
+        __device__ __forceinline__ void h_load_split(u64 (&x)[32], const u64 *__restrict__ rowp, int tid, u64 p, u64 cr1)
+        {
+            static_assert(REDUCE == kTreatNone || REDUCE == kTreatBarrett || REDUCE == kTreatCondSub, "mod-up treatments only");
+            const int jb = Arr<T, 1>::tid_index(tid);
+#pragma unroll
+            for (int batch = 0; batch < 16 / kLoadBatch; batch++)
+            {
+                ulonglong2 a[kLoadBatch], b[kLoadBatch];
+#pragma unroll
+                for (int i = 0; i < kLoadBatch; i++)
+                {
+                    const int idx = jb + Arr<T, 1>::slot_index((batch * kLoadBatch + i) * 2);
+                    a[i] = *reinterpret_cast<const ulonglong2 *>(rowp + 2 * idx);
+                    b[i] = *reinterpret_cast<const ulonglong2 *>(rowp + 2 * idx + 2);
+                }
+#pragma unroll
+                for (int i = 0; i < kLoadBatch; i++)
+                {
+                    const int s = (batch * kLoadBatch + i) * 2;
+                    u64 v0 = HALF ? a[i].y : a[i].x, v1 = HALF ? b[i].y : b[i].x;
+                    if constexpr (REDUCE == kTreatCondSub)
+                    {
+                        v0 = v0 >= p ? v0 - p : v0;
+                        v1 = v1 >= p ? v1 - p : v1;
+                    }
+                    else if constexpr (REDUCE == kTreatBarrett)
+                    {
+                        v0 = barrett_reduce_63(v0, p, cr1);
+                        v1 = barrett_reduce_63(v1, p, cr1);
+                    }
+                    x[s] = v0;
+                    x[s + 1] = v1;
+                }
+                __builtin_amdgcn_sched_barrier(0);
+            }
+        }
+
         template <int T>
         __device__ __forceinline__ void h_store_rows(const u64 (&x)[32], u64 *__restrict__ halfp, int tid)
         {
@@ -616,14 +654,15 @@
             note_nonzero(tflag, 0, nz);
         }
 
-        template <int LOGN, int STRICT, int REDUCE>
+        template <int LOGN, int STRICT, int REDUCE, bool SPLIT = false>
         __global__ __launch_bounds__(1 << (LOGN - 6), 4) void ntt_fwd_half_kernel(
             u64 *__restrict__ data, const PrimeDev *__restrict__ primes, RowMap map, std::size_t nrows, int flags,
             unsigned *__restrict__ tickets, unsigned *__restrict__ timeout_flag, unsigned spin_limit, NttSource src,
             std::size_t chunk, LiveSlots live)
         {
             constexpr int T = LOGN - 1;
-            constexpr int N = 1 << LOGN;
+            constexpr int N = SPLIT ? 1 << (LOGN - 1) : 1 << LOGN;
+            static_assert(!SPLIT || ((STRICT == kSchedLazy || STRICT == kSchedApprox) && REDUCE <= kTreatCondSub), "kFwdSplitInstances");
             extern __shared__ u64 lds[];
             const int wave_base = __builtin_amdgcn_readfirstlane(static_cast<int>(threadIdx.x) & ~63);
             int half, position;
@@ -638,6 +677,8 @@
             const u64 p = P.p, two_p = FP ? fp_bits(P.p_d) : P.two_p, rdp = P.rdp;
             const u64 *tw = FP ? reinterpret_cast<const u64 *>(P.fwd_d) : P.fwd;
             u64 *rowp = data + (row << LOGN);
+            if constexpr (SPLIT)
+                rowp += half << T;
             u64 x[32];
 
             const u64 neg_p = FP ? fp_bits(P.pinv_d) : 0 - p;
@@ -662,12 +703,19 @@
                     x[s] = v.x;
                     x[s + 1] = v.y;
                 }
+            }
+            else if constexpr (SPLIT)
+            {
+                if (half)
+                    h_load_split<T, 1, REDUCE>(x, srcp, fresh_tid(wave_base), p, P.cr1);
+                else
+                    h_load_split<T, 0, REDUCE>(x, srcp, fresh_tid(wave_base), p, P.cr1);
             }
             else if (half)
                 h_load_top<T, STRICT, 1, REDUCE>(x, srcp, tw, fresh_tid(wave_base), two_p, neg_p, P.cr1, src.aux_p, src.aux_cr1, src.aux_top);
             else
                 h_load_top<T, STRICT, 0, REDUCE>(x, srcp, tw, fresh_tid(wave_base), two_p, neg_p, P.cr1, src.aux_p, src.aux_cr1, src.aux_top);
-            const int gbase = half << T;
+            const int gbase = SPLIT ? 0 : half << T;
             u64 w0[kIL], ws0[kIL];
             RoundStage<T, 1, STRICT, true, 0>::load(w0, ws0, tw, gbase, N);
             if constexpr (FP)
@@ -722,7 +770,7 @@
             constexpr int SX = XCH ? 1 : (kStoreSwap<T, REDUCE> ? 2 : 0);
             if constexpr (!XCH)
                 wait_for_sibling();
-            const int fin = ((flags & kNttCanonical) ? 1 : 0) | (((flags & kNttAnyRep) || STRICT == kSchedDense) ? 2 : 0) | ((flags & kNttSmallQuot) ? 4 : 0);
+            const int fin = ((flags & kNttCanonical) ? 1 : 0) | (((flags & kNttAnyRep) || STRICT == kSchedDense || SPLIT) ? 2 : 0) | ((flags & kNttSmallQuot) ? 4 : 0);
             const u64 rdp_fin =
                 ((STRICT == kSchedApprox && (flags & kNttSmallQuot)) || STRICT == kSchedDense) ? static_cast<u64>(__float_as_uint(small_quot_const(p))) : rdp;
             constexpr bool ROUT = REDUCE == kTreatReduceOut || REDUCE == kTreatReduceOutTopDone;
@@ -774,6 +822,45 @@
         {
             return fwd_kernels<LOGN>(std::make_integer_sequence<int, kFwdInstanceCount>{});
         }
+        template <int LOGN, int... I>
+        const FwdKernel *fwd_split_kernels(std::integer_sequence<int, I...>)
+        {
+            static const FwdKernel table[] = { &ntt_fwd_half_kernel<LOGN, kFwdSplitInstances[I].sched, kFwdSplitInstances[I].treatment, true>... };
+            return table;
+        }
+        template <int LOGN>
+        const FwdKernel *fwd_split_kernels()
+        {
+            return fwd_split_kernels<LOGN>(std::make_integer_sequence<int, kFwdSplitInstanceCount>{});
+        }
+
+        FwdChoice choose_fwd(const Engine &e, const RowMap &map, int flags, const NttSource &src, const LiveSlots &live)
+        {
+            u64 live_p[kMaxRows];
+            FwdFacts f{};
+            f.logn = e.logn;
+            f.flags = flags;
+            f.live = live_p;
+            f.live_n = live.n;
+            f.gathers = src.base[0] != nullptr;
+            f.all_gathered = f.same_source = f.key_moduli_fp = true;
+            for (int i = 0; i < live.n; i++)
+            {
+                live_p[i] = e.tables[map.prime[live.slot[i]]].p;
+                if (f.gathers)
+                {
+                    f.all_gathered = f.all_gathered && src.code[live.slot[i]] != kSkipRow;
+                    f.same_source = f.same_source && ((src.code[live.slot[i]] ^ src.code[live.slot[0]]) & ~kSrcReduce) == 0;
+                }
+            }
+            for (std::size_t i = 0; f.gathers && f.key_moduli_fp && i < e.key_moduli.size(); i++)
+                f.key_moduli_fp = e.key_moduli[i] < bounds::kFpInputBound;
+            f.treatment = src.reduce_mode;
+            f.aux_p = src.aux_p;
+            f.sw = ntt_switches();
+            f.suppress_signal = e.ntt_suppress_signal;
+            return select_fwd_half(f);
+        }
 
         template <int LOGN>
         hipError_t launch_half(const Engine &e, u64 *data, std::size_t nrows, const RowMap &map, int flags,
@@ -799,30 +886,7 @@
             const std::size_t blocks = chunk * 16;
             if (blocks > 0x7fffffffull)
                 return hipErrorInvalidValue;
-            u64 live_p[kMaxRows];
-            FwdFacts f{};
-            f.logn = LOGN;
-            f.flags = flags;
-            f.live = live_p;
-            f.live_n = live.n;
-            f.gathers = src.base[0] != nullptr;
-            f.all_gathered = f.same_source = f.key_moduli_fp = true;
-            for (int i = 0; i < live.n; i++)
-            {
-                live_p[i] = e.tables[map.prime[live.slot[i]]].p;
-                if (f.gathers)
-                {
-                    f.all_gathered = f.all_gathered && src.code[live.slot[i]] != kSkipRow;
-                    f.same_source = f.same_source && ((src.code[live.slot[i]] ^ src.code[live.slot[0]]) & ~kSrcReduce) == 0;
-                }
-            }
-            for (std::size_t i = 0; f.gathers && f.key_moduli_fp && i < e.key_moduli.size(); i++)
-                f.key_moduli_fp = e.key_moduli[i] < bounds::kFpInputBound;
-            f.treatment = src.reduce_mode;
-            f.aux_p = src.aux_p;
-            f.sw = ntt_switches();
-            f.suppress_signal = e.ntt_suppress_signal;
-            const FwdChoice c = select_fwd_half(f);
+            const FwdChoice c = choose_fwd(e, map, flags, src, live);
             if (!c.valid)
                 return hipErrorInvalidValue;
             unsigned *tickets = c.tickets ? e.ntt_tickets(nrows) : nullptr;
@@ -839,7 +903,7 @@
                 std::memcpy(&ksrc.aux_top[2], &c2, 8);
             }
             ProfScope prof(e, "ntt_fwd_half", transformed_rows(nrows, map));
-            fwd_kernels<LOGN>()[c.instance]<<<static_cast<unsigned>(blocks), 1 << (LOGN - 6), lds_bytes, e.lane().stream>>>(
+            (c.split ? fwd_split_kernels<LOGN>() : fwd_kernels<LOGN>())[c.instance]<<<static_cast<unsigned>(blocks), 1 << (LOGN - 6), lds_bytes, e.lane().stream>>>(
                 data, e.d_primes, map, nrows, c.flags, tickets, e.lane().d_fault, e.ntt_spin_limit, ksrc, chunk, live);
             return hipGetLastError();
         }
@@ -855,6 +919,12 @@
                     if (err != hipSuccess)
                         return err;
                 }
+            for (int i = 0; i < kFwdSplitInstanceCount; i++)
+            {
+                const hipError_t err = hipFuncSetAttribute(reinterpret_cast<const void *>(fwd_split_kernels<LOGN>()[i]), hipFuncAttributeMaxDynamicSharedMemorySize, lds_bytes);
+                if (err != hipSuccess)
+                    return err;
+            }
             return hipSuccess;
         }
     }
@@ -868,6 +938,15 @@
         case 16: return launch_half<16>(e, data, nrows, map, flags, src);
         default: return hipErrorInvalidValue;
         }
+    }
+
+    bool ntt_fwd_half_splits(const Engine &e, const RowMap &map, int flags, const NttSource &src)
+    {
+        const LiveSlots live = live_slots(map);
+        if (e.logn < 14 || e.logn > 16 || live.n == 0)
+            return false;
+        const FwdChoice c = choose_fwd(e, map, flags | kNttSplitLast, src, live);
+        return c.valid && c.split;
     }
 
     hipError_t ntt_fwd_half_init()
diff --git a/gemini-seal_amd/csrc/ntt_half.hpp b/gemini-seal_amd/csrc/ntt_half.hpp
--- a/gemini-seal_amd/csrc/ntt_half.hpp
+++ b/gemini-seal_amd/csrc/ntt_half.hpp
@@ -13,6 +13,7 @@
                                              const NttSource &src);
     SEALHIP_INTERNAL hipError_t ntt_inv_half(const Engine &e, u64 *data, std::size_t nrows, const RowMap &map, int flags,
                                              const u64 *src = nullptr, std::size_t src_poly_stride = 0);
+    SEALHIP_INTERNAL bool ntt_fwd_half_splits(const Engine &e, const RowMap &map, int flags, const NttSource &src);
     SEALHIP_INTERNAL hipError_t ntt_inv_tensor(const Engine &e, u64 *data, std::size_t nrows, const RowMap &map, int flags,
                                                const u64 *x, std::size_t item_stride, std::size_t poly_stride, int kb,
                                                bool square);
diff --git a/gemini-seal_amd/csrc/ntt_select.hpp b/gemini-seal_amd/csrc/ntt_select.hpp
--- a/gemini-seal_amd/csrc/ntt_select.hpp
+++ b/gemini-seal_amd/csrc/ntt_select.hpp
@@ -15,6 +15,7 @@
     constexpr int kNttDebugNoSignal = 0x40;
     constexpr int kNttTopDone = 0x80;
     constexpr int kNttDeferTop = 4;
+    constexpr int kNttSplitLast = 0x100;
     constexpr bounds::u64 kFpPrimeBound = bounds::u64(1) << bounds::kFpPrimeBits;
 
     constexpr int kSchedLazy = 0;
@@ -77,6 +78,19 @@
         return -1;
     }
 
+    constexpr FwdInstance kFwdSplitInstances[] = {
+        { kSchedLazy, kTreatNone },   { kSchedLazy, kTreatBarrett },   { kSchedLazy, kTreatCondSub },
+        { kSchedApprox, kTreatNone }, { kSchedApprox, kTreatBarrett }, { kSchedApprox, kTreatCondSub },
+    };
+    constexpr int kFwdSplitInstanceCount = static_cast<int>(sizeof(kFwdSplitInstances) / sizeof(kFwdSplitInstances[0]));
+    constexpr int fwd_split_instance_index(int sched, int treatment)
+    {
+        for (int i = 0; i < kFwdSplitInstanceCount; i++)
+            if (kFwdSplitInstances[i].sched == sched && kFwdSplitInstances[i].treatment == treatment)
+                return i;
+        return -1;
+    }
+
     struct InvInstance
     {
         int shape, sched;
@@ -141,6 +155,7 @@
         int flags;
         bool tickets;
         bool aux_as_doubles;
+        bool split;
     };
 
     template <int LOGN>
@@ -166,6 +181,9 @@
         if (top_done && (((flags & (kNttReduceOut | kNttStrict | kNttCanonical)) != kNttReduceOut && !dense) || f.gathers))
             return c;
         const bool all_gathered = f.gathers && f.all_gathered;
+        const bool split = (flags & kNttSplitLast) != 0;
+        if (split && (!all_gathered || (flags & (kNttCanonical | kNttReduceOut | kNttTopDone)) != 0))
+            return c;
         c.tickets = !(top_done || all_gathered);
         if (f.suppress_signal)
             flags |= kNttDebugNoSignal;
@@ -218,6 +236,15 @@
         c.treatment = red;
         c.flags = flags;
         c.aux_as_doubles = fp && f.gathers && special;
+        if (split)
+        {
+            if (fp || !every_live([&](bounds::u64 p) { return bounds::fwd_split_admits(p, LOGN, 1); }))
+                return c;
+            c.split = true;
+            c.instance = fwd_split_instance_index(c.sched, c.treatment);
+            c.valid = c.instance >= 0;
+            return c;
+        }
         c.instance = fwd_instance_index(LOGN, c.sched, c.treatment);
         c.valid = c.instance >= 0;
         return c;
diff --git a/gemini-seal_amd/csrc/pipeline.cpp b/gemini-seal_amd/csrc/pipeline.cpp
--- a/gemini-seal_amd/csrc/pipeline.cpp
+++ b/gemini-seal_amd/csrc/pipeline.cpp
@@ -175,9 +175,10 @@
         {
             const u64 *inb;
             std::size_t inb_stride;
+            bool split_last;
         };
         KsRows ks_digits(Engine &e, LevelTools &lt, int k, const u64 *tg, std::size_t target_stride, std::size_t m, u64 *coeff,
-                         u64 *ext, int dj0, int dj1)
+                         u64 *ext, int dj0, int dj1, bool split_last = false, bool plan_only = false)
         {
             const KsDev &h = lt.h_ks;
             const std::size_t N = e.n;
@@ -190,7 +191,7 @@
             const std::size_t ext_digit = ext_item * m;
             const u64 *src = tg;
             std::size_t src_stride = target_stride;
-            if (ckks)
+            if (ckks && !plan_only)
             {
                 if (ntt_can_gather(e))
                     check(launch_intt_from(e, coeff, tg, target_stride, m * k, map_q, kNttCanonical | kNttAnyRep),
@@ -221,33 +222,45 @@
                 if (bounds::fwd_lazy_admits(pmax, e.logn))
                     modup_mode = kTreatNone;
             }
-            if (!gather)
+            if (!gather && !plan_only)
                 check(launch_ks_modup(e, lt.d_ks, h, src, src_stride, ext, ext_item, ext_digit, m, -1), "modup");
-            for (int j = dj0; j < dj1; j++)
-            {
+            const auto digit_map = [&](int j) {
                 RowMap mj = map_rows;
                 const int r0 = j * e.nsp, r1 = std::min(r0 + e.nsp, k);
                 for (int r = r0; r < r1; r++)
                     mj.prime[r] = kSkipRow;
+                return mj;
+            };
+            const auto digit_source = [&](int j) {
+                NttSource ns{};
+                ns.base[0] = src;
+                ns.poly_stride[0] = src_stride;
+                ns.reduce_mode = modup_mode;
+                const u64 p_src = e.key_moduli[h.row_prime[j]];
+                for (int r = 0; r < rows; r++)
+                {
+                    if (r == j)
+                    {
+                        ns.code[r] = kSkipRow;
+                        continue;
+                    }
+                    const u64 p_dst = e.key_moduli[h.row_prime[r]];
+                    ns.code[r] = static_cast<unsigned short>(j | (p_src <= p_dst ? 0 : kSrcReduce));
+                }
+                return ns;
+            };
+            const int digit_flags = kNttAnyRep | kNttApprox;
+            split_last = split_last && gather && ks_mac_has_pair_form(e, h, m, dj0, dj1);
+            for (int j = dj0; split_last && j < dj1; j++)
+                split_last = ntt_can_split_last(e, digit_map(j), digit_source(j), digit_flags, h.nd);
+            if (plan_only)
+                return KsRows{ nullptr, 0, split_last };
+            for (int j = dj0; j < dj1; j++)
+            {
+                const RowMap mj = digit_map(j);
                 if (gather)
-                {
-                    NttSource ns{};
-                    ns.base[0] = src;
-                    ns.poly_stride[0] = src_stride;
-                    ns.reduce_mode = modup_mode;
-                    const u64 p_src = e.key_moduli[h.row_prime[j]];
-                    for (int r = 0; r < rows; r++)
-                    {
-                        if (r == j)
-                        {
-                            ns.code[r] = kSkipRow;
-                            continue;
-                        }
-                        const u64 p_dst = e.key_moduli[h.row_prime[r]];
-                        ns.code[r] = static_cast<unsigned short>(j | (p_src <= p_dst ? 0 : kSrcReduce));
-                    }
-                    check(launch_ntt_gather(e, ext + j * ext_digit, m * rows, mj, ns, kNttAnyRep | kNttApprox), "ntt(ext, gathered)");
-                }
+                    check(launch_ntt_gather(e, ext + j * ext_digit, m * rows, mj, digit_source(j), digit_flags | (split_last ? kNttSplitLast : 0)),
+                          "ntt(ext, gathered)");
                 else
                     check(launch_ntt(e, ext + j * ext_digit, m * rows, mj, false, kNttAnyRep), "ntt(ext)");
             }
@@ -272,16 +285,16 @@
                 inb = coeff;
                 inb_stride = static_cast<std::size_t>(k) * N;
             }
-            return KsRows{ inb, inb_stride };
+            return KsRows{ inb, inb_stride, split_last };
         }
 
         void ks_products(Engine &e, LevelTools &lt, int k, const u64 *tg, std::size_t target_stride, std::size_t m, u64 *coeff,
                          u64 *ext, const KSwitchKey &key, u64 *prod, int dj0, int dj1)
         {
             const std::size_t ext_item = static_cast<std::size_t>(k + e.nsp) * e.n;
-            const KsRows in_bundle = ks_digits(e, lt, k, tg, target_stride, m, coeff, ext, dj0, dj1);
+            const KsRows in_bundle = ks_digits(e, lt, k, tg, target_stride, m, coeff, ext, dj0, dj1, true);
             check(launch_ks_mac(e, lt.d_ks, lt.h_ks, in_bundle.inb, in_bundle.inb_stride, ext, ext_item, ext_item * m ,
-                                key.d_data, prod, 2 * ext_item, m, dj0, dj1),
+                                key.d_data, prod, 2 * ext_item, m, dj0, dj1, in_bundle.split_last),
                   "mac");
         }
 
@@ -397,6 +410,13 @@
             check(launch_ks_moddown_rescale_post(e, lt.d_ksr, h, base, base_stride, acc, ext_item, temp, out, 2 * m),
                   "moddown_rescale_post");
         }
+    }
+
+    bool ks_split_last_plan(Engine &e, int k, std::size_t count)
+    {
+        LevelTools &lt = e.level(k);
+        const u64 *const rows_not_read = reinterpret_cast<const u64 *>(&lt);
+        return ks_digits(e, lt, k, rows_not_read, 0, count, const_cast<u64 *>(rows_not_read), nullptr, 0, lt.h_ks.nd, true, true).split_last;
     }
 
     void op_switch_key(Engine &e, int k, u64 *ct, std::size_t ct_stride, const u64 *target, std::size_t target_stride,
diff --git a/gemini-seal_amd/sealhip/__init__.py b/gemini-seal_amd/sealhip/__init__.py
--- a/gemini-seal_amd/sealhip/__init__.py
+++ b/gemini-seal_amd/sealhip/__init__.py
@@ -91,6 +91,8 @@
     "sealhip_debug_rns_constants": [_vp, _u32, _u32, _vp, _sz, C.POINTER(_sz)],
     "sealhip_debug_bfv_multiply_plan": [_vp, _u32, _u32, _u32, _i32, _vp],
     "sealhip_debug_behz_dot_split": [_vp, _u32, C.POINTER(C.c_int32)],
+    "sealhip_debug_ks_split_last": [_vp, _u32, _sz, C.POINTER(C.c_int32)],
+    "sealhip_debug_ntt_split_last": [_vp, _u32, _u32, _i32, _vp, _vp],
     "sealhip_ntt_negacyclic_harvey_lazy": [_vp, _vp, _sz, _u32, _u32],
     "sealhip_ntt_negacyclic_harvey": [_vp, _vp, _sz, _u32, _u32],
     "sealhip_inverse_ntt_negacyclic_harvey_lazy": [_vp, _vp, _sz, _u32, _u32],
@@ -565,6 +567,14 @@
         _check(lib().sealhip_debug_behz_dot_split(self.handle, k, C.byref(v)))
         return v.value
 
+    def debug_ks_split_last(self, k, count):
+        v = C.c_int32()
+        _check(lib().sealhip_debug_ks_split_last(self.handle, k, count, C.byref(v)))
+        return bool(v.value)
+
+    def debug_ntt_split_last(self, prime_index, src, dst, treatment=0, exact=False):
+        _check(lib().sealhip_debug_ntt_split_last(self.handle, prime_index, treatment, 1 if exact else 0, _ptr(src), _ptr(dst)))
+
     def galois_elt_from_step(self, step):
         v = C.c_uint32()
         _check(lib().sealhip_galois_elt_from_step(self.handle, step, C.byref(v)))
diff --git a/include/sealhip.h b/include/sealhip.h
--- a/include/sealhip.h
+++ b/include/sealhip.h
@@ -89,6 +89,9 @@
 long sealhip_debug_bfv_multiply_plan(sealhip_context *ctx, uint32_t k, uint32_t size_a, uint32_t size_b, int32_t square,
                                      int32_t *out);
 long sealhip_debug_behz_dot_split(sealhip_context *ctx, uint32_t k, int32_t *out);
+long sealhip_debug_ks_split_last(sealhip_context *ctx, uint32_t k, size_t count, int32_t *out);
+long sealhip_debug_ntt_split_last(sealhip_context *ctx, uint32_t prime_index, uint32_t treatment, int32_t exact,
+                                  const uint64_t *src_device, uint64_t *dst_device);
 
 long sealhip_ntt_negacyclic_harvey_lazy(sealhip_context *ctx, uint64_t *data, size_t count, uint32_t k,
                                         uint32_t base);
```

After: 24590 (median of 6 runs). 1.01x the previous value.
